# algbio/founderblockgraphs

Measured on AMD Instinct MI355X. Metric: MSA columns segmented/sec, higher is better.
Workload: dtype u32

## Files before the change

### founderblockgraphs_amd/csrc/ctx.hip

```cpp
#include "fbg_internal.h"
#include <chrono>
#include <stdarg.h>
#include <stdio.h>
#include <ctype.h>
#include <string.h>
#include <algorithm>
#include <atomic>
#include <thread>
#include <vector>

static std::string g_global_err;

int fbg_fail(fbg_ctx *ctx, int code, const char *fmt, ...)
{
    char buf[1024];
    va_list ap;
    va_start(ap, fmt);
    vsnprintf(buf, sizeof(buf), fmt, ap);
    va_end(ap);
    if (ctx) ctx->err = buf; else g_global_err = buf;
    return code;
}

int fbg_reserve(fbg_ctx *ctx, DevBuf &b, size_t bytes)
{
    if (bytes == 0) bytes = 256;
    if (b.cap >= bytes) return FBG_OK;
    const auto t_begin = std::chrono::steady_clock::now();
    if (b.p) {
        FBG_HIP_TRY(ctx, hipStreamSynchronize(ctx->stream));
        FBG_HIP_TRY(ctx, hipFree(b.p));
        ctx->held_bytes -= b.cap;
        b.p = nullptr; b.cap = 0;
    }
    size_t want = (bytes + 255) & ~(size_t)255;
    hipError_t e = hipMalloc(&b.p, want);
    if (e != hipSuccess) {
        b.p = nullptr;
        return fbg_fail(ctx, FBG_ERR_OOM, "hipMalloc(%zu bytes) failed: %s (context already holds %llu bytes)",
                        want, hipGetErrorString(e), (unsigned long long)ctx->held_bytes);
    }
    b.cap = want;
    ctx->held_bytes += want;
    ctx->alloc_calls++;
    ctx->alloc_us += (uint64_t)std::chrono::duration_cast<std::chrono::microseconds>(std::chrono::steady_clock::now() - t_begin).count();
    if (ctx->opt.poison) FBG_HIP_TRY(ctx, hipMemsetAsync(b.p, (int)(ctx->opt.poison & 255), want, ctx->stream));
    return FBG_OK;
}

void fbg_release(fbg_ctx *ctx, DevBuf &b)
{
    if (b.p) {
        (void)hipFree(b.p);
        ctx->held_bytes -= b.cap;
        b.p = nullptr; b.cap = 0;
    }
}

#define FBG_STAGE_SLOT (8u << 20)
#define FBG_STAGE_SLOTS 16
#define FBG_STAGE_MIN (32u << 20)

static bool host_pointer_is_pinned(const void *p)
{
    hipPointerAttribute_t at;
    const hipError_t e = hipPointerGetAttributes(&at, p);
    if (e != hipSuccess) { (void)hipGetLastError(); return false; }
    return at.type == hipMemoryTypeHost;
}

static int stager_ready(fbg_ctx *ctx)
{
    Stager &s = ctx->stager;
    if (s.base) return FBG_OK;
    FBG_HIP_TRY(ctx, hipHostMalloc(&s.base, (size_t)FBG_STAGE_SLOT * FBG_STAGE_SLOTS, hipHostMallocDefault));
    s.slot_bytes = FBG_STAGE_SLOT; s.nslots = FBG_STAGE_SLOTS;
    s.ev = new hipEvent_t[s.nslots];
    for (int i = 0; i < s.nslots; i++) FBG_HIP_TRY(ctx, hipEventCreateWithFlags(&s.ev[i], hipEventDisableTiming));
    FBG_HIP_TRY(ctx, hipStreamCreateWithFlags(&s.stream, hipStreamNonBlocking));
    return FBG_OK;
}

static int staged_copy(fbg_ctx *ctx, void *dst, const void *src, size_t bytes, bool to_device)
{
    FBG_HIP_TRY(ctx, hipSetDevice(ctx->device));
    FBG_HIP_TRY(ctx, hipStreamSynchronize(ctx->stream));
    const void *host = to_device ? src : dst;
    if (bytes < FBG_STAGE_MIN || host_pointer_is_pinned(host)) {
        FBG_HIP_TRY(ctx, hipMemcpyAsync(dst, src, bytes, to_device ? hipMemcpyHostToDevice : hipMemcpyDeviceToHost, ctx->stream));
        FBG_HIP_TRY(ctx, hipStreamSynchronize(ctx->stream));
        return FBG_OK;
    }
    FBG_TRY(stager_ready(ctx));
    Stager &s = ctx->stager;
    const size_t nchunks = (bytes + s.slot_bytes - 1) / s.slot_bytes;
    unsigned hw = std::thread::hardware_concurrency();
    int T = (int)std::min<size_t>(std::min<unsigned>(std::max(2u, hw / 2), 8u), nchunks);
    if (T > s.nslots / 2) T = s.nslots / 2;
    std::atomic<int> failed{0};
    auto worker = [&](int t) {
        if (hipSetDevice(ctx->device) != hipSuccess) { failed = 1; return; }
        const int slots[2] = {t, t + T};
        uint8_t *pins[2] = {static_cast<uint8_t *>(s.base) + (size_t)slots[0] * s.slot_bytes,
                            static_cast<uint8_t *>(s.base) + (size_t)slots[1] * s.slot_bytes};
        if (to_device) {
            size_t k = 0;
            for (size_t c = (size_t)t; c < nchunks && !failed; c += (size_t)T, k++) {
                const int w = (int)(k & 1);
                const size_t off = c * s.slot_bytes, len = std::min(s.slot_bytes, bytes - off);
                if (k >= 2 && hipEventSynchronize(s.ev[slots[w]]) != hipSuccess) { failed = 1; return; }
                memcpy(pins[w], static_cast<const uint8_t *>(src) + off, len);
                if (hipMemcpyAsync(static_cast<uint8_t *>(dst) + off, pins[w], len, hipMemcpyHostToDevice, s.stream) != hipSuccess ||
                    hipEventRecord(s.ev[slots[w]], s.stream) != hipSuccess) { failed = 1; return; }
            }
        } else {
            auto issue = [&](size_t c, int w) {
                const size_t off = c * s.slot_bytes, len = std::min(s.slot_bytes, bytes - off);
                return hipMemcpyAsync(pins[w], static_cast<const uint8_t *>(src) + off, len, hipMemcpyDeviceToHost, s.stream) == hipSuccess &&
                       hipEventRecord(s.ev[slots[w]], s.stream) == hipSuccess;
            };
            if ((size_t)t < nchunks && !issue((size_t)t, 0)) { failed = 1; return; }
            size_t k = 0;
            for (size_t c = (size_t)t; c < nchunks && !failed; c += (size_t)T, k++) {
                const int w = (int)(k & 1);
                if (c + (size_t)T < nchunks && !issue(c + (size_t)T, w ^ 1)) { failed = 1; return; }
                if (hipEventSynchronize(s.ev[slots[w]]) != hipSuccess) { failed = 1; return; }
                const size_t off = c * s.slot_bytes, len = std::min(s.slot_bytes, bytes - off);
                memcpy(static_cast<uint8_t *>(dst) + off, pins[w], len);
            }
        }
    };
    std::vector<std::thread> th;
    for (int t = 1; t < T; t++) th.emplace_back(worker, t);
    worker(0);
    for (auto &t : th) t.join();
    FBG_HIP_TRY(ctx, hipStreamSynchronize(s.stream));
    if (failed) return fbg_fail(ctx, FBG_ERR_HIP, "staged %s copy of %zu bytes failed: %s", to_device ? "host-to-device" : "device-to-host",
                                bytes, hipGetErrorString(hipGetLastError()));
    return FBG_OK;
}

int fbg_upload(fbg_ctx *ctx, void *d_dst, const void *h_src, size_t bytes) { return staged_copy(ctx, d_dst, h_src, bytes, true); }
int fbg_download(fbg_ctx *ctx, void *h_dst, const void *d_src, size_t bytes) { return staged_copy(ctx, h_dst, d_src, bytes, false); }

int fbg_stage_begin(fbg_ctx *ctx, int stage)
{
    StageTimer &t = ctx->timers[stage];
    if (!t.start) {
        FBG_HIP_TRY(ctx, hipEventCreate(&t.start));
        FBG_HIP_TRY(ctx, hipEventCreate(&t.stop));
    }
    t.recorded = false;
    FBG_HIP_TRY(ctx, hipEventRecord(t.start, ctx->stream));
    return FBG_OK;
}

int fbg_stage_end(fbg_ctx *ctx, int stage, int launches)
{
    StageTimer &t = ctx->timers[stage];
    FBG_HIP_TRY(ctx, hipEventRecord(t.stop, ctx->stream));
    t.recorded = true;
    t.launches = launches;
    return FBG_OK;
}

struct OptKey { const char *name; int64_t FbgOptions::*field; };
static const OptKey g_opt_keys[] = {
    {"no_ranked", &FbgOptions::no_ranked}, {"no_packed", &FbgOptions::no_packed}, {"force_wide", &FbgOptions::force_wide},
    {"full_keys", &FbgOptions::full_keys}, {"no_msd_sort", &FbgOptions::no_msd_sort}, {"msd_min", &FbgOptions::msd_min},
    {"bp_min", &FbgOptions::bp_min}, {"record_scatter", &FbgOptions::record_scatter}, {"lcp_text", &FbgOptions::lcp_text},
    {"no_aux_stream", &FbgOptions::no_aux_stream}, {"rank_no_threshold", &FbgOptions::rank_no_threshold},
    {"dp_literal", &FbgOptions::dp_literal}, {"dp_wave", &FbgOptions::dp_wave}, {"dp_safe_window", &FbgOptions::dp_safe_window},
    {"dp_tile", &FbgOptions::dp_tile}, {"pure_scan", &FbgOptions::pure_scan}, {"gapped_rank", &FbgOptions::gapped_rank}, {"part_tricks_off", &FbgOptions::part_tricks_off}, {"msd_sample_bins", &FbgOptions::msd_sample_bins}, {"msd_min_force", &FbgOptions::msd_min_force}, {"msd_probe", &FbgOptions::msd_probe}, {"msd_xcd", &FbgOptions::msd_xcd}, {"rank_no_lean", &FbgOptions::rank_no_lean}, {"no_stream_upload", &FbgOptions::no_stream_upload},
    {"span_scan", &FbgOptions::span_scan}, {"span_key_flags", &FbgOptions::span_key_flags}, {"span_slow_split", &FbgOptions::span_slow_split}, {"poison", &FbgOptions::poison}, {"dpw_matrix", &FbgOptions::dpw_matrix}, {"dp_chain1", &FbgOptions::dp_chain1},
};

static void options_from_env(FbgOptions &o)
{
    auto env = [](const std::string &name) -> const char * { return getenv(name.c_str()); };
    const char *dbg = env("FBG_DEBUG_ENV");
    if (!dbg || strcmp(dbg, "1") != 0) return;
    for (const OptKey &k : g_opt_keys) {
        std::string name = "FBG_";
        for (const char *c = k.name; *c; c++) name += (char)toupper((unsigned char)*c);
        if (const char *v = env(name)) o.*(k.field) = *v ? strtoll(v, nullptr, 10) : 1;
    }
}

extern "C" {

int fbg_set_option(fbg_ctx *ctx, const char *key, int64_t value)
{
    if (!ctx || !key) return FBG_ERR_INVALID;
    for (const OptKey &k : g_opt_keys)
        if (strcmp(k.name, key) == 0) { ctx->opt.*(k.field) = value; return FBG_OK; }
    return fbg_fail(ctx, FBG_ERR_INVALID, "fbg_set_option: unknown key '%s'", key);
}

int fbg_get_option(const fbg_ctx *ctx, const char *key, int64_t *value)
{
    if (!ctx || !key || !value) return FBG_ERR_INVALID;
    for (const OptKey &k : g_opt_keys)
        if (strcmp(k.name, key) == 0) { *value = ctx->opt.*(k.field); return FBG_OK; }
    if (strcmp(key, "grs_threshold") == 0) { *value = ctx->grs_t; return FBG_OK; }
    if (strcmp(key, "grs_redone") == 0) { *value = (int64_t)ctx->grs_redone; return FBG_OK; }
    if (strcmp(key, "dp_kind") == 0) { *value = ctx->dp_kind; return FBG_OK; }
    if (strcmp(key, "msd_decline") == 0) { *value = ctx->msd_decline; return FBG_OK; }
    if (strcmp(key, "pass1_ahead") == 0) { *value = ctx->pass1_ahead; return FBG_OK; }
    if (strcmp(key, "alloc_calls") == 0) { *value = (int64_t)ctx->alloc_calls; return FBG_OK; }
    if (strcmp(key, "alloc_us") == 0) { *value = (int64_t)ctx->alloc_us; return FBG_OK; }
    if (strcmp(key, "span_decline") == 0) { *value = ctx->sp_decline; return FBG_OK; }
    if (strcmp(key, "span_key_flags_used") == 0) { *value = (ctx->index_valid && ctx->granked && ctx->spanned && ctx->sp_key_flags_sorted) ? 1 : 0; return FBG_OK; }
    if (strcmp(key, "span_scan_used") == 0) { *value = (ctx->index_valid && ctx->granked && ctx->spanned) ? 1 : 0; return FBG_OK; }
    if (strcmp(key, "span_scan_work") == 0) { *value = (int64_t)ctx->sp_work; return FBG_OK; }
    if (strcmp(key, "span_groups") == 0) { *value = (int64_t)ctx->sp_G; return FBG_OK; }
    if (strcmp(key, "span_odd_groups") == 0) { *value = (int64_t)ctx->sp_n_odd[0] + ctx->sp_n_odd[1] + ctx->sp_n_odd[2] + ctx->sp_n_odd[3]; return FBG_OK; }
    if (strcmp(key, "span_irregular") == 0) { *value = (int64_t)ctx->sp_n_irr; return FBG_OK; }
    if (strcmp(key, "span_chain") == 0) { *value = (int64_t)ctx->sp_chain_n; return FBG_OK; }
    if (strcmp(key, "span_slow_groups") == 0) { *value = (int64_t)ctx->sp_slow_n; return FBG_OK; }
    if (strncmp(key, "span_dbg", 8) == 0 && key[8] >= '0' && key[8] <= '7' && !key[9]) {
        unsigned long long v = 0;
        if (hipStreamSynchronize(ctx->stream) != hipSuccess || ctx->scalars.cap < 256 * 8 ||
            hipMemcpy(&v, (const unsigned long long *)ctx->scalars.p + 208 + 24 + (key[8] - '0'), 8, hipMemcpyDeviceToHost) != hipSuccess) return FBG_ERR_HIP;
        *value = (int64_t)v;
        return FBG_OK;
    }
    if (strcmp(key, "index_kind") == 0) {
        *value = !ctx->index_valid ? -1 : ctx->part_active ? 3 : ctx->granked ? 2 : ctx->ranked ? 1 : 0;
        return FBG_OK;
    }
    return FBG_ERR_INVALID;
}

void *fbg_host_alloc(uint64_t bytes)
{
    void *p = nullptr;
    if (hipHostMalloc(&p, bytes ? bytes : 1, hipHostMallocDefault) != hipSuccess) { (void)hipGetLastError(); return nullptr; }
    return p;
}
void fbg_host_free(void *p) { if (p) (void)hipHostFree(p); }

int fbg_ctx_create(int device, fbg_ctx **out)
{
    if (!out) return FBG_ERR_INVALID;
    *out = nullptr;
    int count = 0;
    hipError_t e = hipGetDeviceCount(&count);
    if (e != hipSuccess || count <= 0)
        return fbg_fail(nullptr, FBG_ERR_NO_DEVICE,
                        "no HIP device visible (%s); libfbg_hip has no CPU fallback",
                        e != hipSuccess ? hipGetErrorString(e) : "device count 0");
    if (device < 0 || device >= count)
        return fbg_fail(nullptr, FBG_ERR_INVALID, "device %d out of range (0..%d)", device, count - 1);
    e = hipSetDevice(device);
    if (e != hipSuccess) return fbg_fail(nullptr, FBG_ERR_HIP, "hipSetDevice: %s", hipGetErrorString(e));
    fbg_ctx *ctx = new fbg_ctx();
    ctx->device = device;
    options_from_env(ctx->opt);
    e = hipStreamCreateWithFlags(&ctx->stream, hipStreamNonBlocking);
    if (e != hipSuccess) {
        delete ctx;
        return fbg_fail(nullptr, FBG_ERR_HIP, "hipStreamCreate: %s", hipGetErrorString(e));
    }
    ctx->own_stream = true;
    *out = ctx;
    return FBG_OK;
}

void fbg_ctx_destroy(fbg_ctx *ctx)
{
    if (!ctx) return;
    (void)hipSetDevice(ctx->device);
    (void)hipStreamSynchronize(ctx->stream);
    DevBuf *bufs[] = {&ctx->msa_own, &ctx->text, &ctx->pos, &ctx->tot, &ctx->segtab, &ctx->exc_scratch, &ctx->prow, &ctx->igrow, &ctx->rec,
                      &ctx->xlist, &ctx->gmax, &ctx->excol, &ctx->xslot, &ctx->xbits, &ctx->exc, &ctx->colT, &ctx->keysA, &ctx->keysB, &ctx->valsA, &ctx->valsB, &ctx->grp, &ctx->flags,
                      &ctx->list, &ctx->tie_list, &ctx->big_groups, &ctx->kargs, &ctx->msd_w, &ctx->msd_v, &ctx->tmp, &ctx->small, &ctx->scalars, &ctx->dp_a, &ctx->dp_b, &ctx->dp_c,
                      &ctx->dp_d, &ctx->dp_e, &ctx->dp_f, &ctx->dp_g, &ctx->dp_h, &ctx->io_a, &ctx->io_b,
                      &ctx->io_c, &ctx->io_d, &ctx->bt_up, &ctx->bt_dep, &ctx->ps_a, &ctx->ps_b, &ctx->ps_c, &ctx->ps_d,
                      &ctx->ps_e, &ctx->ps_f, &ctx->ps_g, &ctx->ps_h, &ctx->gwin, &ctx->gbits, &ctx->gwin_rows,
                      &ctx->sp_cells, &ctx->sp_flagT, &ctx->sp_cwin, &ctx->sp_tiles, &ctx->sp_gstart, &ctx->sp_gcol, &ctx->sp_gflags, &ctx->sp_rstart, &ctx->sp_rid,
                      &ctx->sp_gplo, &ctx->sp_gphi, &ctx->sp_gval, &ctx->sp_odd, &ctx->sp_irr, &ctx->sp_chain, &ctx->sp_slow, &ctx->sp_mins};
    for (DevBuf *b : bufs) fbg_release(ctx, *b);
    if (ctx->up_stream) {
        (void)hipStreamSynchronize(ctx->up_stream);
        for (auto &e : ctx->up_ev) if (e) (void)hipEventDestroy(e);
        (void)hipStreamDestroy(ctx->up_stream);
    }
    for (auto &t : ctx->timers) {
        if (t.start) (void)hipEventDestroy(t.start);
        if (t.stop) (void)hipEventDestroy(t.stop);
    }
    if (ctx->stager.base) {
        for (int i = 0; i < ctx->stager.nslots; i++) (void)hipEventDestroy(ctx->stager.ev[i]);
        delete[] ctx->stager.ev;
        (void)hipStreamDestroy(ctx->stager.stream);
        (void)hipHostFree(ctx->stager.base);
    }
    if (ctx->aux_fork) (void)hipEventDestroy(ctx->aux_fork);
    if (ctx->aux_join) (void)hipEventDestroy(ctx->aux_join);
    if (ctx->aux) (void)hipStreamDestroy(ctx->aux);
    if (ctx->own_stream) (void)hipStreamDestroy(ctx->stream);
    delete ctx;
}

const char *fbg_last_error(const fbg_ctx *ctx) { return ctx ? ctx->err.c_str() : g_global_err.c_str(); }

int fbg_set_stream(fbg_ctx *ctx, void *hip_stream)
{
    if (!ctx) return FBG_ERR_INVALID;
    FBG_HIP_TRY(ctx, hipStreamSynchronize(ctx->stream));
    if (ctx->own_stream) { (void)hipStreamDestroy(ctx->stream); ctx->own_stream = false; }
    if (hip_stream) {
        ctx->stream = (hipStream_t)hip_stream;
    } else {
        FBG_HIP_TRY(ctx, hipStreamCreateWithFlags(&ctx->stream, hipStreamNonBlocking));
        ctx->own_stream = true;
    }
    return FBG_OK;
}

int fbg_stage_ms(fbg_ctx *ctx, int stage, float *ms, int *launches)
{
    if (!ctx || stage < 0 || stage >= FBG_STAGE_COUNT) return FBG_ERR_INVALID;
    StageTimer &t = ctx->timers[stage];
    if (ms) *ms = 0.f;
    if (launches) *launches = 0;
    if (!t.recorded) return FBG_OK;
    FBG_HIP_TRY(ctx, hipEventSynchronize(t.stop));
    float v = 0.f;
    FBG_HIP_TRY(ctx, hipEventElapsedTime(&v, t.start, t.stop));
    if (ms) *ms = v;
    if (launches) *launches = t.launches;
    return FBG_OK;
}

uint64_t fbg_device_bytes(const fbg_ctx *ctx) { return ctx ? ctx->held_bytes : 0; }

int fbg_release_scratch(fbg_ctx *ctx)
{
    if (!ctx) return FBG_ERR_INVALID;
    FBG_HIP_TRY(ctx, hipSetDevice(ctx->device));
    FBG_HIP_TRY(ctx, hipStreamSynchronize(ctx->stream));
    const bool sorted_in_A = (ctx->ranked || ctx->granked) && ctx->rk_keys == ctx->keysA.as<uint64_t>();
    DevBuf *bufs[] = {sorted_in_A ? &ctx->keysB : &ctx->keysA, &ctx->valsA, &ctx->grp, &ctx->flags, &ctx->list, &ctx->tie_list, &ctx->msd_w, &ctx->msd_v,
                      &ctx->tmp, &ctx->dp_a, &ctx->dp_b, &ctx->dp_c, &ctx->dp_d, &ctx->dp_e, &ctx->dp_f,
                      &ctx->dp_g, &ctx->dp_h, &ctx->ps_a, &ctx->ps_b, &ctx->ps_c, &ctx->ps_d, &ctx->ps_e, &ctx->ps_f,
                      &ctx->ps_g, &ctx->ps_h, &ctx->sp_cells, &ctx->sp_flagT, &ctx->sp_tiles};
    for (DevBuf *b : bufs) fbg_release(ctx, *b);
    return FBG_OK;
}

int fbg_sync(fbg_ctx *ctx)
{
    if (!ctx) return FBG_ERR_INVALID;
    FBG_HIP_TRY(ctx, hipStreamSynchronize(ctx->stream));
    return FBG_OK;
}

static int check_dims(fbg_ctx *ctx, uint64_t m, uint64_t n)
{
    if (!ctx) return FBG_ERR_INVALID;
    if (m == 0 || n == 0) return fbg_fail(ctx, FBG_ERR_INVALID, "empty MSA (m=%llu, n=%llu)",
                                          (unsigned long long)m, (unsigned long long)n);
    if (n >= (1ull << 31) || m * (n + 1) + 1 >= (1ull << 40))
        return fbg_fail(ctx, FBG_ERR_TOO_LARGE, "MSA of %llu x %llu cells is beyond this engine (n < 2^31, text < 2^40)",
                        (unsigned long long)m, (unsigned long long)n);
    return FBG_OK;
}

int fbg_msa_set_device(fbg_ctx *ctx, const uint8_t *d_msa, uint64_t m, uint64_t n)
{
    FBG_TRY(check_dims(ctx, m, n));
    if (!d_msa) return fbg_fail(ctx, FBG_ERR_INVALID, "null MSA pointer");
    ctx->d_msa = d_msa; ctx->m = m; ctx->n = n; ctx->index_valid = false;
    return FBG_OK;
}

int fbg_msa_load_host(fbg_ctx *ctx, const uint8_t *msa, uint64_t m, uint64_t n)
{
    FBG_TRY(check_dims(ctx, m, n));
    if (!msa) return fbg_fail(ctx, FBG_ERR_INVALID, "null MSA pointer");
    FBG_HIP_TRY(ctx, hipSetDevice(ctx->device));
    FBG_TRY(fbg_reserve(ctx, ctx->msa_own, m * n));
    FBG_TRY(fbg_upload(ctx, ctx->msa_own.p, msa, m * n));
    ctx->d_msa = ctx->msa_own.as<uint8_t>(); ctx->m = m; ctx->n = n; ctx->index_valid = false;
    return FBG_OK;
}

int fbg_index_build(fbg_ctx *ctx, int reversed, const uint8_t *ignore_chars, uint64_t ignore_len)
{
    if (!ctx) return FBG_ERR_INVALID;
    if (!ctx->d_msa) return fbg_fail(ctx, FBG_ERR_INVALID, "fbg_index_build: no MSA set");
    FBG_HIP_TRY(ctx, hipSetDevice(ctx->device));
    for (int st : {FBG_STAGE_SORT_PASS1, FBG_STAGE_SORT_PASS2, FBG_STAGE_SORT_PASS3, FBG_STAGE_RANK_KERNEL}) {
        ctx->timers[st].recorded = false;
        ctx->timers[st].launches = 0;
    }
    ctx->index_valid = false;
    ctx->granked = false;
    ctx->spanned = false;
    ctx->gpart = false;
    ctx->reversed = reversed ? 1 : 0;
    FBG_TRY(fbg_build_text(ctx, reversed ? nullptr : ignore_chars, reversed ? 0 : ignore_len));
    FBG_TRY(fbg_suffix_sort(ctx));
    FBG_TRY(fbg_neighbour_lcp(ctx));
    if (ctx->N > 1500000000ull) {
        size_t free_b = 0, total_b = 0;
        FBG_HIP_TRY(ctx, hipMemGetInfo(&free_b, &total_b));
        if (free_b < total_b / 2) FBG_TRY(fbg_release_scratch(ctx));
    }
    ctx->index_valid = true;
    return FBG_OK;
}

int fbg_part_index_build(fbg_ctx *ctx, int reversed, int part, int nparts, void *d_blob, int *ok)
{
    return fbg_part_index_build_ignore(ctx, reversed, part, nparts, nullptr, 0, d_blob, ok);
}

int fbg_part_index_build_ignore(fbg_ctx *ctx, int reversed, int part, int nparts, const uint8_t *ignore_chars, uint64_t ignore_len, void *d_blob, int *ok)
{
    if (!ctx) return FBG_ERR_INVALID;
    if (!ctx->d_msa) return fbg_fail(ctx, FBG_ERR_INVALID, "fbg_part_index_build: no MSA set");
    if (!d_blob || !ok || nparts < 1 || part < 0 || part >= nparts || (ignore_len && !ignore_chars))
        return fbg_fail(ctx, FBG_ERR_INVALID, "fbg_part_index_build: bad arguments");
    FBG_HIP_TRY(ctx, hipSetDevice(ctx->device));
    ctx->index_valid = false;
    ctx->ranked = false;
    ctx->granked = false;
    ctx->spanned = false;
    ctx->reversed = reversed ? 1 : 0;
    ctx->gpart = false;
    ctx->allow_wide = true;
    const int rc = fbg_build_text(ctx, reversed ? nullptr : ignore_chars, reversed ? 0 : ignore_len);
    ctx->allow_wide = false;
    FBG_TRY(rc);
    return fbg_part_sort(ctx, part, nparts, static_cast<uint8_t *>(d_blob), ok);
}

int fbg_part_scan(fbg_ctx *ctx, const void *d_blobs, uint32_t *d_gmax, int *ok)
{
    if (!ctx) return FBG_ERR_INVALID;
    if (!ctx->part_active || ctx->index_valid)
        return fbg_fail(ctx, FBG_ERR_INVALID, "fbg_part_scan needs fbg_part_index_build first");
    if (!d_blobs || !d_gmax || !ok) return fbg_fail(ctx, FBG_ERR_INVALID, "fbg_part_scan: bad arguments");
    FBG_HIP_TRY(ctx, hipSetDevice(ctx->device));
    if (ctx->gpart) return fbg_grs_part_scan(ctx, static_cast<const uint8_t *>(d_blobs), d_gmax, ok);
    return fbg_rank_part_runs(ctx, static_cast<const uint8_t *>(d_blobs), d_gmax, ok);
}

int fbg_part_finish(fbg_ctx *ctx, const uint32_t *d_gmax, int *ok)
{
    if (!ctx) return FBG_ERR_INVALID;
    if (!ctx->part_active || ctx->index_valid)
        return fbg_fail(ctx, FBG_ERR_INVALID, "fbg_part_finish needs fbg_part_scan first");
    if (!d_gmax || !ok) return fbg_fail(ctx, FBG_ERR_INVALID, "fbg_part_finish: bad arguments");
    FBG_HIP_TRY(ctx, hipSetDevice(ctx->device));
    uint32_t verdict = 1;
    FBG_HIP_TRY(ctx, hipMemcpyAsync(ctx->gmax.p, d_gmax, (ctx->n + 1) * 4, hipMemcpyDeviceToDevice, ctx->stream));
    FBG_HIP_TRY(ctx, hipMemcpyAsync(&verdict, d_gmax + ctx->n, 4, hipMemcpyDeviceToHost, ctx->stream));
    FBG_HIP_TRY(ctx, hipStreamSynchronize(ctx->stream));
    *ok = verdict == 0;
    if (*ok) {
        uint64_t unfilled = 0;
        if (ctx->gpart) FBG_TRY(fbg_grs_part_unfilled(ctx, &unfilled));
        else FBG_TRY(fbg_rank_part_unfilled(ctx, &unfilled));
        if (unfilled) { *ok = 2; return FBG_OK; }
        ctx->n_exc = 0; ctx->index_valid = true;
        if (ctx->gpart) ctx->granked = true; else ctx->ranked = true;
    }
    return FBG_OK;
}

int fbg_part_rescan(fbg_ctx *ctx, uint32_t *d_gmax)
{
    if (!ctx) return FBG_ERR_INVALID;
    if (!ctx->part_active || ctx->index_valid)
        return fbg_fail(ctx, FBG_ERR_INVALID, "fbg_part_rescan follows a fbg_part_finish that returned *ok = 2");
    if (!d_gmax) return fbg_fail(ctx, FBG_ERR_INVALID, "fbg_part_rescan: bad arguments");
    FBG_HIP_TRY(ctx, hipSetDevice(ctx->device));
    uint32_t verdict = 0;
    if (ctx->gpart) { FBG_TRY(fbg_grs_part_rescan(ctx)); verdict = ctx->grs_part_failed ? 1u : 0u; }
    else FBG_TRY(fbg_rank_part_rescan(ctx));
    FBG_HIP_TRY(ctx, hipMemcpyAsync(d_gmax, ctx->gmax.p, (ctx->n + 1) * 4, hipMemcpyDeviceToDevice, ctx->stream));
    FBG_HIP_TRY(ctx, hipMemcpyAsync(d_gmax + ctx->n, &verdict, 4, hipMemcpyHostToDevice, ctx->stream));
    FBG_HIP_TRY(ctx, hipStreamSynchronize(ctx->stream));
    return FBG_OK;
}

int fbg_scan_f(fbg_ctx *ctx, uint64_t x0, uint64_t x1, int disable_tricks, uint64_t *d_f)
{
    if (!ctx) return FBG_ERR_INVALID;
    if (!ctx->index_valid || ctx->reversed)
        return fbg_fail(ctx, FBG_ERR_INVALID, "fbg_scan_f needs fbg_index_build(reversed=0) first");
    if (x0 > x1 || x1 > ctx->n || !d_f) return fbg_fail(ctx, FBG_ERR_INVALID, "fbg_scan_f: bad column range");
    FBG_HIP_TRY(ctx, hipSetDevice(ctx->device));
    return fbg_scan_columns(ctx, x0, x1, FBG_SCAN_F, disable_tricks, d_f);
// ... 238 lines not shown
```

### founderblockgraphs_amd/csrc/fbg_internal.h

```cpp
#pragma once
#include <cstring>
#include <cstdlib>
#include <hip/hip_runtime.h>
#include <stdint.h>
#include <string>
#include "../../include/fbg_hip.h"

#define FBG_WAVE 64

struct DevBuf {
    void *p = nullptr;
    size_t cap = 0;
    template <class T> T *as() const { return reinterpret_cast<T *>(p); }
};

struct Stager {
    void *base = nullptr;
    size_t slot_bytes = 0;
    int nslots = 0;
    hipEvent_t *ev = nullptr;
    hipStream_t stream = nullptr;
};

struct StageTimer {
    hipEvent_t start = nullptr, stop = nullptr;
    bool recorded = false;
    int launches = 0;
};

struct FbgOptions {
    int64_t no_ranked = 0, no_packed = 0, force_wide = 0, full_keys = 0, no_msd_sort = 0, msd_min = -1, bp_min = -1,
            record_scatter = 0, lcp_text = 0, no_aux_stream = 0, rank_no_threshold = 0, dp_literal = 0, dp_wave = 0,
            dp_safe_window = 0, dp_tile = 0, pure_scan = 0, gapped_rank = 0, part_tricks_off = 0, msd_sample_bins = 0, msd_min_force = 0, msd_probe = 0, msd_xcd = -1, rank_no_lean = 0, no_stream_upload = 0,
            span_scan = 0, span_key_flags = 0, span_slow_split = 0, poison = 0, dpw_matrix = 0, dp_chain1 = 0;
};

struct fbg_ctx {
    int device = 0;
    FbgOptions opt;
    hipStream_t stream = nullptr;
    bool own_stream = false;
    hipStream_t aux = nullptr;
    hipEvent_t aux_fork = nullptr, aux_join = nullptr;
    bool aux_pending = false;
    std::string err;
    uint64_t held_bytes = 0;
    Stager stager;

    const uint8_t *d_msa = nullptr;
    DevBuf msa_own;
    uint64_t m = 0, n = 0;

    const uint8_t *up_host = nullptr;
    hipStream_t up_stream = nullptr;
    hipEvent_t up_ev[9] = {};
    bool pre_pass1 = false;
    uint64_t pre_symbols[4] = {0, 0, 0, 0};
    alignas(16) unsigned char pre_state[768];
    uint64_t pre_tiles = 0;
    int pass1_ahead = 0;

    bool index_valid = false;
    int reversed = 0;
    bool gapfree = true;
    bool have_ignore = false;
    uint64_t N = 0;
    uint64_t byte_hist[256] = {0};
    bool allow_wide = false;
    uint32_t mp = 0;
    DevBuf text;
    DevBuf pos, tot;
    DevBuf segtab;
    DevBuf prow;
    DevBuf igrow;
    DevBuf rec;
    uint32_t *sa_ptr = nullptr;
    bool lcp_from_keys = false;
    DevBuf colT;
    DevBuf xlist;
    bool ranked = false;
    DevBuf gmax, excol, xslot;
    DevBuf xbits;
    DevBuf exc_scratch;
    DevBuf exc;
    uint32_t n_exc = 0;
    bool granked = false;
    int grs_tricks_off = 0;
    bool grs_skip = false;
    uint32_t grs_ign_lo = 0, grs_ign_hi = 0;
    DevBuf gwin;
    DevBuf gbits;
    DevBuf gwin_rows;
    const uint64_t *grs_ebits = nullptr;
    bool grs_flagged = false;
    bool pairs_similar = false;
    bool grs_ties_done = false;
    bool gpart = false;
    bool grs_part_failed = false;
    uint32_t grs_t = 1;
    uint64_t grs_redone = 0;
    bool spanned = false;
    DevBuf sp_cells;
    DevBuf sp_flagT;
    bool sp_key_flags = false;
    uint64_t alloc_calls = 0, alloc_us = 0;
    int sp_decline = 0;
    bool sp_key_flags_sorted = false;
    DevBuf sp_cwin;
    DevBuf sp_tiles, sp_gstart, sp_gcol, sp_gflags, sp_rstart, sp_rid, sp_gplo, sp_gphi, sp_gval, sp_odd, sp_irr, sp_chain, sp_slow, sp_mins;
    uint32_t sp_chain_n = 0, sp_slow_n = 0;
    uint64_t sp_G = 0, sp_R = 0, sp_n_irr = 0, sp_work = 0;
    uint32_t sp_n_odd[4] = {0, 0, 0, 0}, sp_odd_cap = 0;
    const uint32_t *sort_payload = nullptr;
    int64_t msd_decline = -1;
    int dp_kind = -1;
    bool cells_built = false;
    uint8_t ignore_tab[256] = {0};
    uint64_t *rk_keys = nullptr;
    int rk_b = 0, rk_key_bits = 0, rk_K = 0;
    int rk_layout = 0, rk_pb = 0;
    bool part_active = false;
    int part = 0, nparts = 1;
    uint64_t part_count = 0;
    uint64_t part_T = 0;
    uint32_t part_gmin = 0;

    DevBuf keysA, keysB, valsA, valsB, grp, flags, list, tie_list, big_groups, tmp, small, scalars;
    DevBuf kargs;
    alignas(16) unsigned char kargs_host[512];
    DevBuf msd_w, msd_v;
    DevBuf dp_a, dp_b, dp_c, dp_d, dp_e, dp_f, dp_g, dp_h, io_a, io_b, io_c, io_d;
    DevBuf bt_up, bt_dep;
    DevBuf ps_a, ps_b, ps_c, ps_d, ps_e, ps_f, ps_g, ps_h;

    StageTimer timers[FBG_STAGE_COUNT];
};

int fbg_fail(fbg_ctx *ctx, int code, const char *fmt, ...);
#define FBG_HIP_TRY(ctx, expr)                                                              \
    do {                                                                                    \
        hipError_t e_ = (expr);                                                             \
        if (e_ != hipSuccess)                                                               \
            return fbg_fail((ctx), e_ == hipErrorOutOfMemory ? FBG_ERR_OOM : FBG_ERR_HIP,   \
                            "%s failed: %s (%s:%d)", #expr, hipGetErrorString(e_), __FILE__, \
                            __LINE__);                                                      \
    } while (0)
#define FBG_TRY(expr)                \
    do {                             \
        int rc_ = (expr);            \
        if (rc_ != FBG_OK) return rc_; \
    } while (0)

int fbg_reserve(fbg_ctx *ctx, DevBuf &b, size_t bytes);
int fbg_upload(fbg_ctx *ctx, void *d_dst, const void *h_src, size_t bytes);
int fbg_download(fbg_ctx *ctx, void *h_dst, const void *d_src, size_t bytes);
void fbg_release(fbg_ctx *ctx, DevBuf &b);
int fbg_stage_begin(fbg_ctx *ctx, int stage);
int fbg_stage_end(fbg_ctx *ctx, int stage, int launches);

#define FBG_SLOTS_PAIRS 0
#define FBG_SLOTS_PACKED 1
#define FBG_SLOTS_WIDE 2
struct KeyGeom {
    int b = 0, K = 0, key_bits = 0;
    bool compact = false, packed = false;
    bool wide = false;
    int pb = 0;
    const uint8_t *d_code = nullptr;
};

int fbg_build_text(fbg_ctx *ctx, const uint8_t *ignore, uint64_t ignore_len);
int fbg_suffix_sort(fbg_ctx *ctx);
int fbg_neighbour_lcp(fbg_ctx *ctx);
int fbg_rank_scan_try(fbg_ctx *ctx, uint64_t *keys, uint32_t *vals, const KeyGeom &g, int *done);
int fbg_pure_scan_try(fbg_ctx *ctx, uint64_t *keys, uint32_t *vals, const KeyGeom &g, int *done);
int fbg_rank_finish(fbg_ctx *ctx, uint64_t x0, uint64_t x1, int mode, int disable_tricks, uint64_t *d_out);
int fbg_rank_materialize(fbg_ctx *ctx, uint32_t *d_sa, uint32_t *d_isa, uint32_t *d_pl, uint32_t *d_pr);
#define FBG_STAGE_RANKSCAN FBG_STAGE_TILE
int fbg_grs_prepare(fbg_ctx *ctx, int *launches);
int fbg_grs_part_classify(fbg_ctx *ctx, uint64_t *keys, uint32_t *vals, uint64_t count, const KeyGeom &g, int eligible, uint8_t *d_blob, int *ok);
int fbg_grs_part_scan(fbg_ctx *ctx, const uint8_t *d_blobs, uint32_t *d_gmax, int *ok);
int fbg_grs_part_unfilled(fbg_ctx *ctx, uint64_t *unfilled);
int fbg_grs_part_rescan(fbg_ctx *ctx);
int fbg_grs_strip(fbg_ctx *ctx, uint32_t *vals);
int fbg_grs_try(fbg_ctx *ctx, uint64_t *keys, uint32_t *vals, const KeyGeom &g, int *done);
int fbg_grs_finish(fbg_ctx *ctx, uint64_t x0, uint64_t x1, int disable_tricks, uint64_t *d_out, int *ok);
int fbg_grs_materialize(fbg_ctx *ctx, uint32_t *d_sa, uint32_t *d_isa, uint32_t *d_pl, uint32_t *d_pr);
bool fbg_span_eligible(fbg_ctx *ctx, const KeyGeom &g);
bool fbg_span_key_flags(fbg_ctx *ctx, KeyGeom &g);
int fbg_span_prepare(fbg_ctx *ctx, const KeyGeom &g, int *launches);
int fbg_span_try(fbg_ctx *ctx, uint64_t *keys, uint32_t *vals, const KeyGeom &g, int *done);
int fbg_span_rescan(fbg_ctx *ctx, int disable_tricks, int *ok);
int fbg_build_cell_tables(fbg_ctx *ctx);
int fbg_key_setup(fbg_ctx *ctx, bool compact, KeyGeom *g, int *launches);
int fbg_rank_part_classify(fbg_ctx *ctx, uint64_t *keys, uint32_t *vals, uint64_t count, const KeyGeom &g, int pre_ok,
                           uint8_t *d_blob, int *ok);
int fbg_rank_part_runs(fbg_ctx *ctx, const uint8_t *d_blobs, uint32_t *d_gmax, int *ok);
int fbg_rank_part_unfilled(fbg_ctx *ctx, uint64_t *unfilled);
int fbg_rank_part_rescan(fbg_ctx *ctx);
int fbg_part_sort(fbg_ctx *ctx, int part, int nparts, uint8_t *d_blob, int *ok);
int fbg_msd_sort(fbg_ctx *ctx, const KeyGeom &g, uint64_t **sorted, int *ok, int *launches);
int fbg_msd_pre_begin(fbg_ctx *ctx, int *ok);
int fbg_msd_pre_pass1(fbg_ctx *ctx, uint64_t avail);
bool fbg_msd_pre_geom(fbg_ctx *ctx, KeyGeom *g);
int fbg_msd_sort_part(fbg_ctx *ctx, const KeyGeom &g, uint64_t lo, uint64_t hi, int nohi, int nparts, uint64_t out_offset,
                      uint64_t *count, int *ok, int *launches);
int fbg_sample_sort_pairs(fbg_ctx *ctx, const KeyGeom &g, int *ok, int *launches);
int fbg_scan_columns(fbg_ctx *ctx, uint64_t x0, uint64_t x1, int mode, int disable_tricks,
                     uint64_t *d_out);
int fbg_dp_minmax(fbg_ctx *ctx, const uint64_t *d_f, uint64_t n, uint64_t *d_boundaries,
                  uint64_t *count_out, uint64_t *d_mml, uint64_t *d_bt);
int fbg_dp_repeatfree(fbg_ctx *ctx, const uint64_t *d_v, uint64_t n, uint64_t *d_s,
                      uint64_t *d_prev, uint64_t *d_boundaries, uint64_t *count_out);
int fbg_gapped_v_from_f(fbg_ctx *ctx, const uint64_t *d_f, uint64_t n, uint64_t *d_v);
int fbg_dp_gapped(fbg_ctx *ctx, const uint64_t *d_v, uint64_t n, uint64_t *d_s, uint64_t *d_prev,
                  uint64_t *d_boundaries, uint64_t *count_out);

#define FBG_SCAN_F 0
#define FBG_SCAN_V 1

static inline unsigned fbg_blocks(uint64_t work, unsigned per_block, unsigned cap = 0x7fffffffu)
{
    uint64_t b = (work + per_block - 1) / per_block;
    if (b < 1) b = 1;
    if (b > cap) b = cap;
    return (unsigned)b;
}
```

### founderblockgraphs_amd/csrc/msd_sort.hip

```cpp
#include "fbg_internal.h"
#include "msd_keys.h"
#include <rocprim/rocprim.hpp>
#include <algorithm>
#include <cmath>

#define MSD_DIG 9
#define MSD_NB (1 << MSD_DIG)
#define MSD_THREADS 1024
#define MSD_TILE (MSD_THREADS * MSD_ITEMS)
#define MSD_FN_THREADS 512
#define MSD_FN_CAP 4096
#define MSD_FN_ITEMS (MSD_FN_CAP / MSD_FN_THREADS)
#define MSD_FN_BITS 11
#define MSD_FN_BINS (1 << MSD_FN_BITS)
#define MSD_BIG_THREADS 1024
#define MSD_BIG_CAP 16384
#define MSD_ARENA (1u << 20)

struct MsdArgs {
    const uint8_t *T;
    uint64_t N;
    const uint8_t *code;
    int b, K, pb, kb;
    uint64_t *buf1;
    uint64_t cap1;
    int xs;
    uint64_t segcap;
    unsigned long long *count1;
    const uint32_t *tile_start;
    uint64_t tile0;
    uint32_t tiles2, tiles2_x;
    uint64_t *buf2;
    uint32_t *count2;
    const unsigned long long *off;
    uint64_t *out;
    uint32_t *arena_sb;
    uint64_t *arena_w;
    unsigned long long *arena_count;
    uint32_t arena_cap;
    unsigned long long *flag;
};

__device__ __forceinline__ void msd_scan_and_reserve(uint32_t *cnt, uint32_t *loff, uint32_t *gdelta, uint32_t *wsum,
                                                     unsigned long long *cursor_d, bool wide_cursor, uint32_t *cursor32_d)
{
    const uint32_t lane = threadIdx.x & 63, wv = threadIdx.x >> 6;
    const uint32_t c = threadIdx.x < MSD_NB ? cnt[threadIdx.x] : 0u;
    uint32_t inc = c;
#pragma unroll
    for (int d = 1; d < 64; d <<= 1) { const uint32_t o = __shfl_up(inc, d, 64); if ((int)lane >= d) inc += o; }
    if (lane == 63) wsum[wv] = inc;
    __syncthreads();
    uint32_t pre = 0;
    for (uint32_t q = 0; q < wv; q++) pre += wsum[q];
    if (threadIdx.x < MSD_NB) {
        loff[threadIdx.x] = pre + inc - c;
        unsigned long long g = 0;
        if (c) g = wide_cursor ? atomicAdd(cursor_d, (unsigned long long)c) : (unsigned long long)atomicAdd(cursor32_d, c);
        gdelta[threadIdx.x] = (uint32_t)g - (pre + inc - c);
    }
    __syncthreads();
}

template <bool FULL>
__device__ __forceinline__ void msd_pack_split_body(const MsdArgs &a, uint64_t *buf, const uint8_t *cd, uint32_t *cnt, uint32_t *loff, uint32_t *gdelta,
                                                    uint32_t *wsum)
{
    uint8_t *tile = reinterpret_cast<uint8_t *>(buf);
    const int b = a.b, K = a.K;
    const uint64_t base = ((uint64_t)blockIdx.x + a.tile0) * MSD_TILE;
    msd_load_tile<MSD_TILE, FULL>(tile, cd, a.T, a.N, base);
    __syncthreads();
    const int t0 = threadIdx.x * MSD_ITEMS;
    uint64_t w[MSD_ITEMS];
    msd_build_keys(tile, t0, b, K, w);
    __syncthreads();
    uint32_t rk[MSD_ITEMS];
    const int dshift = a.kb - MSD_DIG;
#pragma unroll
    for (int i = 0; i < MSD_ITEMS; i++) {
        const uint64_t p = base + t0 + i;
        const bool ok = FULL || p < a.N;
        rk[i] = ok ? atomicAdd(&cnt[(uint32_t)(w[i] >> dshift)], 1u) : 0xffffffffu;
        w[i] = (w[i] << a.pb) | p;
    }
    __syncthreads();
    const uint32_t xq = a.xs > 1 ? (blockIdx.x & (uint32_t)(a.xs - 1)) : 0u;
    msd_scan_and_reserve(cnt, loff, gdelta, wsum, a.count1 + (threadIdx.x < MSD_NB ? threadIdx.x * a.xs + xq : 0), true, nullptr);
    const int wshift = a.pb + dshift;
    uint64_t *const obase = a.buf1 + xq * a.segcap;
#pragma unroll
    for (int i = 0; i < MSD_ITEMS; i++)
        if (FULL || rk[i] != 0xffffffffu) buf[loff[(uint32_t)(w[i] >> wshift)] + rk[i]] = w[i];
    __syncthreads();
    const uint32_t have = FULL ? (uint32_t)MSD_TILE : (uint32_t)min((uint64_t)MSD_TILE, a.N - base);
    bool over = false;
#pragma unroll
    for (int r = 0; r < MSD_ITEMS; r++) {
        const uint32_t j = threadIdx.x + r * MSD_THREADS;
        if (FULL || j < have) {
            const uint64_t x = buf[j];
            const uint32_t d = (uint32_t)(x >> wshift);
            const uint32_t at = j + gdelta[d];
            if (at < a.segcap) obase[(uint64_t)d * a.cap1 + at] = x;
            else over = true;
        }
    }
    if (over) atomicOr(a.flag, 2ull);
}

__global__ __launch_bounds__(MSD_THREADS) void k_msd_pack_split(MsdArgs a)
{
    __shared__ uint64_t buf[MSD_TILE];
    __shared__ uint8_t cd[256];
    __shared__ uint32_t cnt[MSD_NB], loff[MSD_NB];
    __shared__ uint32_t gdelta[MSD_NB];
    __shared__ uint32_t wsum[MSD_THREADS / 64];
    if (threadIdx.x < 256) cd[threadIdx.x] = a.code[threadIdx.x];
    if (threadIdx.x < MSD_NB) cnt[threadIdx.x] = 0;
    __syncthreads();
    msd_pack_split_body<false>(a, buf, cd, cnt, loff, gdelta, wsum);
}

__global__ __launch_bounds__(1024) void k_msd_tiles(const unsigned long long *__restrict__ count1, uint64_t segcap, uint32_t nseg,
                                                    uint32_t *__restrict__ tile_start, unsigned long long *__restrict__ flag)
{
    __shared__ uint32_t wsum[16];
    const uint32_t lane = threadIdx.x & 63, wv = threadIdx.x >> 6;
    uint32_t t[4], tot = 0;
#pragma unroll
    for (int q = 0; q < 4; q++) {
        const uint32_t s = threadIdx.x * 4 + q;
        t[q] = 0;
        if (s < nseg) {
            const unsigned long long c = count1[s] < segcap ? count1[s] : segcap;
            if (count1[s] > segcap) atomicOr(flag, 4ull);
            t[q] = (uint32_t)((c + MSD_TILE - 1) / MSD_TILE);
        }
        tot += t[q];
    }
    uint32_t inc = tot;
#pragma unroll
    for (int d = 1; d < 64; d <<= 1) { const uint32_t o = __shfl_up(inc, d, 64); if ((int)lane >= d) inc += o; }
    if (lane == 63) wsum[wv] = inc;
    __syncthreads();
    uint32_t pre = inc - tot;
    for (uint32_t q = 0; q < wv; q++) pre += wsum[q];
#pragma unroll
    for (int q = 0; q < 4; q++) {
        const uint32_t s = threadIdx.x * 4 + q;
        if (s < nseg) tile_start[s] = pre;
        pre += t[q];
        if (s + 1 == nseg) tile_start[nseg] = pre;
    }
}

template <bool FULL>
__device__ __forceinline__ void msd_split_body(const MsdArgs &a, uint64_t *buf, uint32_t *cnt, uint32_t *loff, uint32_t *gdelta, uint32_t *wsum,
                                               const uint64_t *__restrict__ in, uint32_t have, uint32_t seg)
{
    const int wshift = a.pb + a.kb - 2 * MSD_DIG;
    uint64_t w[MSD_ITEMS];
    uint32_t rk[MSD_ITEMS];
#pragma unroll
    for (int r = 0; r < MSD_ITEMS; r++) {
        const uint32_t j = threadIdx.x + r * MSD_THREADS;
        w[r] = (FULL || j < have) ? in[j] : 0ull;
    }
#pragma unroll
    for (int r = 0; r < MSD_ITEMS; r++) {
        const uint32_t j = threadIdx.x + r * MSD_THREADS;
        rk[r] = (FULL || j < have) ? atomicAdd(&cnt[(uint32_t)(w[r] >> wshift) & (MSD_NB - 1)], 1u) : 0u;
    }
    __syncthreads();
    msd_scan_and_reserve(cnt, loff, gdelta, wsum, nullptr, false,
                         a.count2 + (size_t)seg * MSD_NB + (threadIdx.x < MSD_NB ? threadIdx.x : 0));
#pragma unroll
    for (int r = 0; r < MSD_ITEMS; r++) {
        const uint32_t j = threadIdx.x + r * MSD_THREADS;
        if (FULL || j < have) buf[loff[(uint32_t)(w[r] >> wshift) & (MSD_NB - 1)] + rk[r]] = w[r];
    }
    __syncthreads();
    uint64_t *const obase = a.buf2 + (uint64_t)seg * MSD_NB * MSD_FN_CAP;
#pragma unroll
    for (int r = 0; r < MSD_ITEMS; r++) {
        const uint32_t j = threadIdx.x + r * MSD_THREADS;
        if (FULL || j < have) {
            const uint64_t x = buf[j];
            const uint32_t d = (uint32_t)(x >> wshift) & (MSD_NB - 1);
            const uint32_t at = j + gdelta[d];
            if (at < MSD_FN_CAP) obase[d * MSD_FN_CAP + at] = x;
            else {
                const unsigned long long e = atomicAdd(a.arena_count, 1ull);
                if (e < a.arena_cap) { a.arena_sb[e] = seg * MSD_NB + d; a.arena_w[e] = x; }
                else atomicOr(a.flag, 8ull);
            }
        }
    }
}

__global__ __launch_bounds__(MSD_THREADS) void k_msd_split(MsdArgs a)
{
    __shared__ uint64_t buf[MSD_TILE];
    __shared__ uint32_t cnt[MSD_NB], loff[MSD_NB];
    __shared__ uint32_t gdelta[MSD_NB];
    __shared__ uint32_t wsum[MSD_THREADS / 64];
    const uint32_t tile = a.tiles2_x ? (blockIdx.x & 7u) * a.tiles2_x + (blockIdx.x >> 3) : blockIdx.x;
    if (tile >= a.tiles2) return;
    uint32_t lo = 0, hi = MSD_NB * (uint32_t)a.xs;
    while (hi - lo > 1) { const uint32_t mid = (lo + hi) / 2; if (a.tile_start[mid] <= tile) lo = mid; else hi = mid; }
    const uint32_t seg = lo / (uint32_t)a.xs;
    const uint64_t segn = min((uint64_t)a.count1[lo], a.segcap);
    const uint64_t first = (uint64_t)(tile - a.tile_start[lo]) * MSD_TILE;
    const uint32_t have = (uint32_t)min((uint64_t)MSD_TILE, segn - first);
    const uint64_t *in = a.buf1 + (uint64_t)seg * a.cap1 + (uint64_t)(lo % (uint32_t)a.xs) * a.segcap + first;
    if (threadIdx.x < MSD_NB) cnt[threadIdx.x] = 0;
    __syncthreads();
    if (__builtin_amdgcn_readfirstlane((int)have) == MSD_TILE) msd_split_body<true>(a, buf, cnt, loff, gdelta, wsum, in, have, seg);
    else msd_split_body<false>(a, buf, cnt, loff, gdelta, wsum, in, have, seg);
}

__global__ void k_msd_widen(const uint32_t *__restrict__ count2, unsigned long long *__restrict__ wide, uint64_t cnt)
{
    const uint64_t i = (uint64_t)blockIdx.x * blockDim.x + threadIdx.x;
    if (i < cnt) wide[i] = count2[i];
}

#define MSD_BIG_BIN 192
#define MSD_LOW_BITS 10
template <int CAP, int THREADS>
__device__ __forceinline__ void msd_finish_sort(uint64_t *buf, uint32_t *cnt, uint32_t *loff, uint32_t *wsum, uint64_t (&w)[CAP / THREADS],
                                                uint32_t have, int fshift, uint32_t fmask, int lowbits, uint32_t *sub, uint16_t *biglist,
                                                uint32_t *nbig_lds)
{
    constexpr int ITEMS = CAP / THREADS;
    for (int i = threadIdx.x; i < MSD_FN_BINS; i += THREADS) cnt[i] = 0;
    __syncthreads();
    uint32_t rk[ITEMS];
#pragma unroll
    for (int r = 0; r < ITEMS; r++) {
        const uint32_t j = threadIdx.x + r * THREADS;
        rk[r] = j < have ? atomicAdd(&cnt[(uint32_t)(w[r] >> fshift) & fmask], 1u) : 0u;
    }
    __syncthreads();
    {
        constexpr int PER = MSD_FN_BINS / THREADS > 0 ? MSD_FN_BINS / THREADS : 1;
        const uint32_t lane = threadIdx.x & 63, wv = threadIdx.x >> 6;
        const bool mine = threadIdx.x * PER < MSD_FN_BINS;
        uint32_t c[PER], tot = 0;
#pragma unroll
        for (int q = 0; q < PER; q++) { c[q] = mine ? cnt[threadIdx.x * PER + q] : 0u; tot += c[q]; }
        uint32_t inc = tot;
#pragma unroll
        for (int d = 1; d < 64; d <<= 1) { const uint32_t o = __shfl_up(inc, d, 64); if ((int)lane >= d) inc += o; }
        if (lane == 63) wsum[wv] = inc;
        __syncthreads();
        uint32_t pre = inc - tot;
        for (uint32_t q = 0; q < wv; q++) pre += wsum[q];
        if (mine) {
#pragma unroll
            for (int q = 0; q < PER; q++) { loff[threadIdx.x * PER + q] = pre; pre += c[q]; }
        }
    }
    __syncthreads();
#pragma unroll
    for (int r = 0; r < ITEMS; r++) {
        const uint32_t j = threadIdx.x + r * THREADS;
        if (j < have) buf[loff[(uint32_t)(w[r] >> fshift) & fmask] + rk[r]] = w[r];
    }
    __syncthreads();
    uint32_t nbig = 0;
    if (lowbits >= 1 && lowbits <= MSD_LOW_BITS) {
        if (threadIdx.x == 0) *nbig_lds = 0;
        __syncthreads();
        for (int i = threadIdx.x; i < MSD_FN_BINS; i += THREADS)
            if (cnt[i] > MSD_BIG_BIN) { const uint32_t e = atomicAdd(nbig_lds, 1u); biglist[e] = (uint16_t)i; }
        __syncthreads();
        nbig = *nbig_lds;
    }
    const uint32_t lowmask = (1u << (lowbits > 0 ? lowbits : 1)) - 1;
    for (uint32_t e = 0; e < nbig; e++) {
        const uint32_t bbin = biglist[e], b0 = loff[bbin];
        for (uint32_t i = threadIdx.x; i <= lowmask; i += THREADS) sub[i] = 0;
        __syncthreads();
        uint32_t idx[ITEMS];
#pragma unroll
        for (int r = 0; r < ITEMS; r++) {
            const uint32_t j = threadIdx.x + r * THREADS;
            idx[r] = 0;
            if (j < have && ((uint32_t)(w[r] >> fshift) & fmask) == bbin) idx[r] = atomicAdd(&sub[(uint32_t)(w[r] >> (fshift - lowbits)) & lowmask], 1u);
        }
        __syncthreads();
        {
            constexpr int PER = (1 << MSD_LOW_BITS) / THREADS > 0 ? (1 << MSD_LOW_BITS) / THREADS : 1;
            const uint32_t lane = threadIdx.x & 63, wv = threadIdx.x >> 6;
            uint32_t c[PER], tot = 0;
#pragma unroll
            for (int q = 0; q < PER; q++) { const uint32_t i = threadIdx.x * PER + q; c[q] = i <= lowmask ? sub[i] : 0u; tot += c[q]; }
            uint32_t inc = tot;
#pragma unroll
            for (int d = 1; d < 64; d <<= 1) { const uint32_t o = __shfl_up(inc, d, 64); if ((int)lane >= d) inc += o; }
            if (lane == 63) wsum[wv] = inc;
            __syncthreads();
            uint32_t pre = inc - tot;
            for (uint32_t q = 0; q < wv; q++) pre += wsum[q];
#pragma unroll
            for (int q = 0; q < PER; q++) { const uint32_t i = threadIdx.x * PER + q; if (i <= lowmask) sub[i] = pre; pre += c[q]; }
        }
        __syncthreads();
#pragma unroll
        for (int r = 0; r < ITEMS; r++) {
            const uint32_t j = threadIdx.x + r * THREADS;
            if (j < have && ((uint32_t)(w[r] >> fshift) & fmask) == bbin)
                rk[r] = b0 + sub[(uint32_t)(w[r] >> (fshift - lowbits)) & lowmask] + idx[r];
        }
        __syncthreads();
    }
    if (nbig) {
#pragma unroll
        for (int r = 0; r < ITEMS; r++) {
            const uint32_t j = threadIdx.x + r * THREADS;
            if (j < have && cnt[(uint32_t)(w[r] >> fshift) & fmask] > MSD_BIG_BIN) buf[rk[r]] = w[r];
        }
        __syncthreads();
    }
#pragma unroll
    for (int r = 0; r < ITEMS; r++) {
        const uint32_t j = threadIdx.x + r * THREADS;
        if (j < have) {
            const uint64_t y = buf[j];
            const uint32_t bin = (uint32_t)(y >> fshift) & fmask;
            const uint32_t b0 = loff[bin], c = cnt[bin];
            uint32_t at = j;
            if (!(c > MSD_BIG_BIN && (nbig || lowbits == 0))) {
                uint32_t smaller = 0;
                for (uint32_t q = 0; q < c; q++) smaller += buf[b0 + q] < y ? 1u : 0u;
                at = b0 + smaller;
            }
            w[r] = y;
            rk[r] = at;
        }
    }
    __syncthreads();
#pragma unroll
    for (int r = 0; r < ITEMS; r++) {
        const uint32_t j = threadIdx.x + r * THREADS;
        if (j < have) buf[rk[r]] = w[r];
    }
    __syncthreads();
}

template <int CAP, int THREADS>
__device__ __forceinline__ void msd_finish_body(uint64_t *buf, uint32_t *cnt, uint32_t *loff, uint32_t *wsum, const uint64_t *in_a,
                                                uint32_t n_a, const uint64_t *in_b, uint32_t have, uint64_t *out, int fshift,
                                                uint32_t fmask, int lowbits, uint32_t *sub, uint16_t *biglist, uint32_t *nbig_lds)
{
    constexpr int ITEMS = CAP / THREADS;
    uint64_t w[ITEMS];
#pragma unroll
    for (int r = 0; r < ITEMS; r++) {
        const uint32_t j = threadIdx.x + r * THREADS;
        w[r] = j < have ? (j < n_a ? in_a[j] : in_b[j - n_a]) : ~0ull;
    }
    msd_finish_sort<CAP, THREADS>(buf, cnt, loff, wsum, w, have, fshift, fmask, lowbits, sub, biglist, nbig_lds);
#pragma unroll
    for (int r = 0; r < ITEMS; r++) {
        const uint32_t j = threadIdx.x + r * THREADS;
        if (j < have) out[j] = buf[j];
    }
}

__global__ __launch_bounds__(MSD_FN_THREADS) void k_msd_finish(MsdArgs a, int fshift, uint32_t fmask)
{
    __shared__ uint64_t buf[MSD_FN_CAP];
    __shared__ uint32_t cnt[MSD_FN_BINS], loff[MSD_FN_BINS];
    __shared__ uint32_t wsum[MSD_FN_THREADS / 64];
    __shared__ uint32_t sub[1 << MSD_LOW_BITS];
    __shared__ uint16_t biglist[MSD_FN_CAP / MSD_BIG_BIN + 1];
    __shared__ uint32_t nbig_lds;
    const uint32_t have = a.count2[blockIdx.x];
    if (have == 0 || have > MSD_FN_CAP) return;
    const uint64_t *in = a.buf2 + (uint64_t)blockIdx.x * MSD_FN_CAP;
    msd_finish_body<MSD_FN_CAP, MSD_FN_THREADS>(buf, cnt, loff, wsum, in, have, in, have, a.out + a.off[blockIdx.x], fshift, fmask,
                                                fshift - a.pb, sub, biglist, &nbig_lds);
}

__global__ __launch_bounds__(MSD_BIG_THREADS) void k_msd_finish_big(MsdArgs a, const uint32_t *__restrict__ sb_sorted,
                                                                    const uint64_t *__restrict__ w_sorted, uint32_t entries,
                                                                    int fshift, uint32_t fmask)
{
    __shared__ uint64_t buf[MSD_BIG_CAP];
    __shared__ uint32_t cnt[MSD_FN_BINS], loff[MSD_FN_BINS];
    __shared__ uint32_t wsum[MSD_BIG_THREADS / 64];
    __shared__ uint32_t sub[1 << MSD_LOW_BITS];
    __shared__ uint16_t biglist[MSD_BIG_CAP / MSD_BIG_BIN + 1];
    __shared__ uint32_t nbig_lds;
    const uint32_t e = blockIdx.x;
    if (e >= entries) return;
    const uint32_t sb = sb_sorted[e];
    if (e > 0 && sb_sorted[e - 1] == sb) return;
    const uint32_t have = a.count2[sb];
    if (have > MSD_BIG_CAP || have <= MSD_FN_CAP) { if (threadIdx.x == 0) atomicOr(a.flag, 16ull); return; }
    msd_finish_body<MSD_BIG_CAP, MSD_BIG_THREADS>(buf, cnt, loff, wsum, a.buf2 + (uint64_t)sb * MSD_FN_CAP, MSD_FN_CAP, w_sorted + e, have,
                                                  a.out + a.off[sb], fshift, fmask, fshift - a.pb, sub, biglist, &nbig_lds);
}

struct MsdPlan {
    KeyGeom g;
    MsdArgs a;
    uint64_t nsub;
    uint32_t nseg;
    int rest, fbits, xcd;
    uint32_t *tile_start;
    unsigned long long *off, *flag;
};
static_assert(sizeof(MsdPlan) <= sizeof(((fbg_ctx *)nullptr)->pre_state), "room for the plan of a sort begun ahead");

static int msd_plan(fbg_ctx *ctx, const KeyGeom &g, MsdPlan *p, int *ok)
{
    *ok = 0;
    const uint64_t N = ctx->N;
    const int rest = g.key_bits - 2 * MSD_DIG;
    const uint64_t min_n = ctx->opt.msd_min >= 0 ? (uint64_t)ctx->opt.msd_min : (1ull << 24);
    if (!g.packed || !g.compact || N < min_n || rest < 1 || ctx->opt.no_msd_sort) return FBG_OK;
    if (N >= (1ull << 31)) return FBG_OK;
    const int fbits = rest < MSD_FN_BITS ? rest : MSD_FN_BITS;
    if (fbits < 6) return FBG_OK;
    hipStream_t st = ctx->stream;
    const int xcd = ctx->opt.msd_xcd < 0 ? 3 : (int)ctx->opt.msd_xcd;
    const int xs = (xcd & 2) ? 8 : 1;
    const uint64_t cap1 = (N / MSD_NB + N / (4 * MSD_NB) + 65536) & ~127ull;
    const uint64_t nsub = (uint64_t)MSD_NB * MSD_NB;
    if (N / nsub + N / (32 * nsub) + 64 > MSD_FN_CAP) return FBG_OK;
    FBG_TRY(fbg_reserve(ctx, ctx->keysA, (size_t)MSD_NB * cap1 * 8));
    FBG_TRY(fbg_reserve(ctx, ctx->keysB, (size_t)nsub * MSD_FN_CAP * 8));
    const uint32_t nseg = MSD_NB * (uint32_t)xs;
    FBG_TRY(fbg_reserve(ctx, ctx->dp_a, (size_t)nseg * 8 + ((size_t)nseg + 1) * 4 + 64));
    FBG_TRY(fbg_reserve(ctx, ctx->dp_b, nsub * 4));
    FBG_TRY(fbg_reserve(ctx, ctx->dp_c, (nsub + 1) * 8));
    FBG_TRY(fbg_reserve(ctx, ctx->dp_d, (size_t)MSD_ARENA * 4 * 2));
    FBG_TRY(fbg_reserve(ctx, ctx->dp_e, (size_t)MSD_ARENA * 8 * 2));
    unsigned long long *flag = ctx->scalars.as<unsigned long long>() + 100;
    MsdArgs &a = p->a;
    a.T = ctx->text.as<uint8_t>(); a.N = N; a.code = g.d_code; a.b = g.b; a.K = g.K; a.pb = g.pb; a.kb = g.key_bits;
    a.buf1 = ctx->keysA.as<uint64_t>(); a.cap1 = cap1; a.xs = xs; a.segcap = cap1 / xs;
    a.tile0 = 0; a.tiles2 = 0; a.tiles2_x = 0;
    a.count1 = ctx->dp_a.as<unsigned long long>();
    p->tile_start = reinterpret_cast<uint32_t *>(ctx->dp_a.as<uint8_t>() + (size_t)nseg * 8);
    a.tile_start = p->tile_start;
    a.buf2 = ctx->keysB.as<uint64_t>();
    a.count2 = ctx->dp_b.as<uint32_t>();
    p->off = ctx->dp_c.as<unsigned long long>();
    a.off = p->off;
    a.out = ctx->keysA.as<uint64_t>();
    a.flag = flag;
    a.arena_sb = ctx->dp_d.as<uint32_t>(); a.arena_w = ctx->dp_e.as<uint64_t>(); a.arena_count = flag + 1; a.arena_cap = MSD_ARENA;
    p->g = g; p->nsub = nsub; p->nseg = nseg; p->rest = rest; p->fbits = fbits; p->xcd = xcd; p->flag = flag;
    FBG_HIP_TRY(ctx, hipMemsetAsync(flag, 0, 16, st));
    FBG_HIP_TRY(ctx, hipMemsetAsync(a.count1, 0, (size_t)nseg * 8, st));
    FBG_HIP_TRY(ctx, hipMemsetAsync(a.count2, 0, nsub * 4, st));
    *ok = 1;
    return FBG_OK;
}

int fbg_msd_pre_begin(fbg_ctx *ctx, int *ok)
{
    *ok = 0;
    if (ctx->have_ignore || ctx->reversed || ctx->opt.no_ranked) return FBG_OK;
    int launches = 0;
    KeyGeom g;
    FBG_TRY(fbg_key_setup(ctx, true, &g, &launches));
    MsdPlan plan;
    int good = 0;
    FBG_TRY(msd_plan(ctx, g, &plan, &good));
    if (!good) return FBG_OK;
    for (int w = 0; w < 4; w++) ctx->pre_symbols[w] = 0;
    for (int b = 0; b < 256; b++) if (ctx->byte_hist[b]) ctx->pre_symbols[b >> 6] |= 1ull << (b & 63);
    memcpy(ctx->pre_state, &plan, sizeof(plan));
    ctx->pre_tiles = 0;
    *ok = 1;
    return FBG_OK;
}

int fbg_msd_pre_pass1(fbg_ctx *ctx, uint64_t avail)
{
    MsdPlan plan;
    memcpy(&plan, ctx->pre_state, sizeof(plan));
    const uint64_t N = plan.a.N;
    const uint64_t upto = avail >= N ? (N + MSD_TILE - 1) / MSD_TILE : (avail >= 64 ? (avail - 64) / MSD_TILE : 0);
    if (upto <= ctx->pre_tiles) return FBG_OK;
    plan.a.tile0 = ctx->pre_tiles;
    hipLaunchKernelGGL(k_msd_pack_split, dim3((unsigned)(upto - ctx->pre_tiles)), dim3(MSD_THREADS), 0, ctx->stream, plan.a);
    ctx->pre_tiles = upto;
    return FBG_OK;
}

bool fbg_msd_pre_geom(fbg_ctx *ctx, KeyGeom *g)
{
    if (!ctx->pre_pass1) return false;
    MsdPlan plan;
    memcpy(&plan, ctx->pre_state, sizeof(plan));
    *g = plan.g;
    return true;
}

int fbg_msd_sort(fbg_ctx *ctx, const KeyGeom &g, uint64_t **sorted, int *ok, int *launches)
{
    *ok = 0;
    ctx->msd_decline = 1;
    const uint64_t N = ctx->N;
    hipStream_t st = ctx->stream;
    MsdPlan plan;
    const bool ahead = ctx->pre_pass1;
    ctx->pre_pass1 = false;
    ctx->pass1_ahead = ahead ? 1 : 0;
    if (ahead) memcpy(&plan, ctx->pre_state, sizeof(plan));
    else {
        int good = 0;
        FBG_TRY(msd_plan(ctx, g, &plan, &good));
        if (!good) return FBG_OK;
    }
    MsdArgs &a = plan.a;
    const uint64_t nsub = plan.nsub;
    const uint32_t nseg = plan.nseg;
    const int rest = plan.rest, fbits = plan.fbits, xcd = plan.xcd;
    uint32_t *tile_start = plan.tile_start;
    unsigned long long *off = plan.off, *flag = plan.flag;
    if (!ahead) {
        FBG_TRY(fbg_stage_begin(ctx, FBG_STAGE_SORT_PASS1));
        hipLaunchKernelGGL(k_msd_pack_split, dim3(fbg_blocks(N, MSD_TILE)), dim3(MSD_THREADS), 0, st, a);
        FBG_TRY(fbg_stage_end(ctx, FBG_STAGE_SORT_PASS1, 1));
    }
    hipLaunchKernelGGL(k_msd_tiles, dim3(1), dim3(1024), 0, st, a.count1, a.segcap, nseg, tile_start, flag);
    uint32_t tiles2 = 0;
    unsigned long long h_flag = 0;
    FBG_HIP_TRY(ctx, hipMemcpyAsync(&tiles2, tile_start + nseg, 4, hipMemcpyDeviceToHost, st));
    FBG_HIP_TRY(ctx, hipMemcpyAsync(&h_flag, flag, 8, hipMemcpyDeviceToHost, st));
    FBG_HIP_TRY(ctx, hipStreamSynchronize(st));
    *launches += 2;
    ctx->msd_decline = (int64_t)h_flag;
    if (h_flag != 0 || tiles2 == 0) return FBG_OK;
    a.tiles2 = tiles2;
    a.tiles2_x = (xcd & 1) ? (tiles2 + 7) / 8 : 0;
    const unsigned grid2 = a.tiles2_x ? 8 * a.tiles2_x : tiles2;
    FBG_TRY(fbg_stage_begin(ctx, FBG_STAGE_SORT_PASS2));
    hipLaunchKernelGGL(k_msd_split, dim3(grid2), dim3(MSD_THREADS), 0, st, a);
    FBG_TRY(fbg_stage_end(ctx, FBG_STAGE_SORT_PASS2, 1));
    unsigned long long *wide = reinterpret_cast<unsigned long long *>(ctx->keysA.p);
    hipLaunchKernelGGL(k_msd_widen, dim3(fbg_blocks(nsub, 256)), dim3(256), 0, st, a.count2, wide, nsub);
    {
        size_t bytes = 0;
        hipError_t e = rocprim::exclusive_scan(nullptr, bytes, wide, off, 0ull, (size_t)nsub, rocprim::plus<unsigned long long>(), st);
        if (e != hipSuccess) return fbg_fail(ctx, FBG_ERR_HIP, "rocprim scan size query: %s", hipGetErrorString(e));
        FBG_TRY(fbg_reserve(ctx, ctx->tmp, bytes));
        size_t have = ctx->tmp.cap;
        e = rocprim::exclusive_scan(ctx->tmp.p, have, wide, off, 0ull, (size_t)nsub, rocprim::plus<unsigned long long>(), st);
        if (e != hipSuccess) return fbg_fail(ctx, FBG_ERR_HIP, "rocprim exclusive_scan: %s", hipGetErrorString(e));
    }
    const int fshift = g.pb + rest - fbits;
    const uint32_t fmask = (uint32_t)((1u << fbits) - 1);
    FBG_TRY(fbg_stage_begin(ctx, FBG_STAGE_SORT_PASS3));
    hipLaunchKernelGGL(k_msd_finish, dim3((unsigned)nsub), dim3(MSD_FN_THREADS), 0, st, a, fshift, fmask);
    FBG_TRY(fbg_stage_end(ctx, FBG_STAGE_SORT_PASS3, 1));
    unsigned long long h2[2] = {0, 0};
    FBG_HIP_TRY(ctx, hipMemcpyAsync(h2, flag, 16, hipMemcpyDeviceToHost, st));
    FBG_HIP_TRY(ctx, hipStreamSynchronize(st));
    *launches += 4;
    ctx->msd_decline = (int64_t)h2[0];
    if (h2[0] != 0) return FBG_OK;
    if (h2[1] > 0) {
        const uint32_t entries = (uint32_t)h2[1];
        uint32_t *sb_sorted = a.arena_sb + MSD_ARENA;
        uint64_t *w_sorted = a.arena_w + MSD_ARENA;
        size_t bytes = 0;
        hipError_t e = rocprim::radix_sort_pairs(nullptr, bytes, a.arena_sb, sb_sorted, a.arena_w, w_sorted, (size_t)entries, 0u, 32u, st);
        if (e != hipSuccess) return fbg_fail(ctx, FBG_ERR_HIP, "rocprim sort size query: %s", hipGetErrorString(e));
        FBG_TRY(fbg_reserve(ctx, ctx->tmp, bytes));
        size_t have = ctx->tmp.cap;
        e = rocprim::radix_sort_pairs(ctx->tmp.p, have, a.arena_sb, sb_sorted, a.arena_w, w_sorted, (size_t)entries, 0u, 32u, st);
        if (e != hipSuccess) return fbg_fail(ctx, FBG_ERR_HIP, "rocprim radix_sort_pairs: %s", hipGetErrorString(e));
        hipLaunchKernelGGL(k_msd_finish_big, dim3(entries), dim3(MSD_BIG_THREADS), 0, st, a, sb_sorted, w_sorted, entries, fshift, fmask);
        FBG_HIP_TRY(ctx, hipMemcpyAsync(h2, flag, 16, hipMemcpyDeviceToHost, st));
        FBG_HIP_TRY(ctx, hipStreamSynchronize(st));
        *launches += 2;
        ctx->msd_decline = (int64_t)h2[0];
        if (h2[0] != 0) return FBG_OK;
    }
    FBG_HIP_TRY(ctx, hipGetLastError());
    *sorted = ctx->keysA.as<uint64_t>();
    *ok = 1;
    return FBG_OK;
}
```

### founderblockgraphs_amd/csrc/rank_common.h

```cpp
#pragma once
#include "fbg_internal.h"
#include "text_cmp.h"

#define RS_TG 4

__device__ __forceinline__ uint32_t rs_key_lcp(uint64_t a, uint64_t c, int b, int key_bits)
{
    const uint64_t d = a ^ c;
    const uint32_t bits = (uint32_t)(__clzll((long long)d) - (64 - key_bits));
    const uint32_t inv_b = (65536u + (uint32_t)b - 1) / (uint32_t)b;
    return (bits * inv_b) >> 16;
}

struct RankArgs {
    uint32_t magic32;
    uint64_t magic64;
    uint64_t *keys;
    uint32_t *vals;
    uint64_t pmask;
    int pb;
    const uint8_t *T;
    uint64_t N, n;
    uint64_t Ntext;
    uint64_t own_lo, own_hi;
    int first_part, last_part;
    int part_mode;
    int values_only;
    uint32_t row_len;
    uint32_t g_min;
    int b, key_bits, K, reversed;
    uint32_t *gmax;
    uint32_t *cand;
    uint32_t *blk_count;
    uint32_t region;
    uint32_t *ties;
    uint32_t *tie_count;
    uint32_t tie_region;
    uint2 *pairs;
    uint32_t *pair_count;
    uint32_t *pm;
    uint32_t *big;
    unsigned long long *counters;
};

struct Slot {
    uint64_t key;
    uint64_t pos;
    uint32_t col;
    uint32_t rem;
};

__device__ __forceinline__ uint32_t rs_col_of_rem(const RankArgs &a, uint32_t rem)
{
    return rem == 0 ? (uint32_t)a.n : (a.reversed ? rem - 1 : (uint32_t)a.n - rem);
}
template <int L> struct PosT { typedef uint32_t type; };
template <> struct PosT<FBG_SLOTS_WIDE> { typedef uint64_t type; };
template <int L> __device__ __forceinline__ uint64_t rs_key(const RankArgs &a, uint64_t k) { return a.keys[k] >> a.pb; }
template <int L> __device__ __forceinline__ uint64_t rs_pos_of(const RankArgs &a, uint64_t w, uint32_t v)
{
    if (L == FBG_SLOTS_PACKED) return w & a.pmask;
    if (L == FBG_SLOTS_WIDE) return ((w & a.pmask) << 32) | v;
    return v;
}
template <int L> __device__ __forceinline__ uint64_t rs_pos(const RankArgs &a, uint64_t k)
{
    return rs_pos_of<L>(a, L == FBG_SLOTS_PAIRS ? 0ull : a.keys[k], L == FBG_SLOTS_PACKED ? 0u : a.vals[k]);
}
template <int L> __device__ __forceinline__ void rs_set_pos(const RankArgs &a, uint64_t k, uint64_t p)
{
    if (L == FBG_SLOTS_PACKED) a.keys[k] = (a.keys[k] & ~a.pmask) | p;
    else if (L == FBG_SLOTS_WIDE) { a.keys[k] = (a.keys[k] & ~a.pmask) | (p >> 32); a.vals[k] = (uint32_t)p; }
    else a.vals[k] = (uint32_t)p;
}
template <int L> __device__ __forceinline__ uint32_t rs_rem(const RankArgs &a, uint64_t p)
{
    if (L == FBG_SLOTS_WIDE) {
        uint64_t c = p - __umul64hi(p, a.magic64) * a.row_len;
        if (c >= a.row_len) c -= a.row_len;
        return p == a.Ntext - 1 ? 0u : (uint32_t)(a.n - c);
    }
    const uint32_t p32 = (uint32_t)p;
    uint32_t c = p32 - __umulhi(p32, a.magic32) * a.row_len;
    if (c >= a.row_len) c -= a.row_len;
    return p32 == (uint32_t)(a.Ntext - 1) ? 0u : (uint32_t)a.n - c;
}
template <int L> __device__ __forceinline__ Slot rs_slot(const RankArgs &a, uint64_t k)
{
    Slot s;
    const uint64_t w = a.keys[k];
    s.key = w >> a.pb;
    s.pos = rs_pos_of<L>(a, w, L == FBG_SLOTS_PACKED ? 0u : a.vals[k]);
    s.rem = rs_rem<L>(a, s.pos);
    s.col = rs_col_of_rem(a, s.rem);
    return s;
}
template <int L> __device__ __forceinline__ uint32_t rs_col(const RankArgs &a, uint64_t k)
{
    return rs_col_of_rem(a, rs_rem<L>(a, rs_pos<L>(a, k)));
}

__device__ __forceinline__ void rs_update(const RankArgs &a, uint32_t col, uint32_t g)
{
    if (a.gmax[col] < g) atomicMax(&a.gmax[col], g);
}


__device__ __forceinline__ void rs_append(bool want, uint32_t *counter, uint32_t *list, uint32_t region, uint32_t value)
{
    const unsigned long long mask = __ballot(want);
    if (!mask) return;
    const int lane = threadIdx.x & 63;
    uint32_t base = 0;
    const int leader = __ffsll((long long)mask) - 1;
    if (lane == leader) base = atomicAdd(counter, (uint32_t)__popcll(mask));
    base = __shfl(base, leader, 64);
    if (want) {
        const uint32_t slot = base + (uint32_t)__popcll(mask & ((1ull << lane) - 1));
        if (slot < region) list[(size_t)blockIdx.x * region + slot] = value;
    }
}

#define RS_HALO 8

struct RsLdsView {
    const uint64_t *skey;
    const uint32_t *srem;
    __device__ __forceinline__ uint64_t key(int i) const { return skey[i]; }
    __device__ __forceinline__ uint32_t rem(int i) const { return srem[i]; }
};
struct RsWordView {
    const uint64_t *words;
    const RankArgs *a;
    int lo, hi;
    __device__ __forceinline__ uint64_t word(int i) const { return i >= lo && i < hi ? words[i] : 0ull; }
    __device__ __forceinline__ uint64_t key(int i) const { return word(i) >> a->pb; }
    __device__ __forceinline__ uint32_t rem(int i) const { return rs_rem<FBG_SLOTS_PACKED>(*a, word(i) & a->pmask); }
};

template <class V>
__device__ __forceinline__ void rank_scan_slow(const RankArgs &a, const V &v, const int i,
                                               const int lo_i, const int hi_i, const uint64_t k, bool &want_cand, bool &want_tie)
{
    const uint64_t key = v.key(i);
    const uint32_t rem = v.rem(i);
    const bool has_prev = i > lo_i, has_next = i + 1 < hi_i;
    const uint64_t kp = v.key(i - 1), kn = v.key(i + 1);
    const bool tie = (has_prev && kp == key) || (has_next && kn == key);
    if (tie) {
        int h = i, t = i;
        while (h > lo_i && i - h < RS_TG && v.key(h - 1) == key) h--;
        bool big = h > lo_i && v.key(h - 1) == key;
        while (t + 1 < hi_i && t - i < RS_TG && v.key(t + 1) == key) t++;
        big = big || (t + 1 < hi_i && v.key(t + 1) == key) || t - h + 1 > RS_TG;
        bool simple = !big;
        if (simple && a.part_mode && (k - (uint64_t)(i - h) < a.own_lo + 2 || k + (uint64_t)(t - i) + 2 >= a.own_hi))
            simple = false;
        if (simple) {
            uint32_t cols[RS_TG];
            const int s = t - h + 1;
#pragma unroll
            for (int q = 0; q < RS_TG; q++) {
                cols[q] = 0xffffffffu - (uint32_t)q;
                if (q < s) {
                    cols[q] = v.rem(h + q);
                    if (cols[q] < (uint32_t)a.K) simple = false;
                }
            }
#pragma unroll
            for (int q = 0; q < RS_TG; q++)
#pragma unroll
                for (int r = q + 1; r < RS_TG; r++)
                    if (cols[q] == cols[r]) simple = false;
            if (simple && h > lo_i) {
                if (h - 1 > lo_i && v.key(h - 2) == v.key(h - 1)) simple = false;
                const uint32_t oc = v.rem(h - 1);
#pragma unroll
                for (int q = 0; q < RS_TG; q++)
                    if (cols[q] == oc) simple = false;
            }
            if (simple && t + 1 < hi_i) {
                if (t + 2 < hi_i && v.key(t + 2) == v.key(t + 1)) simple = false;
                const uint32_t oc = v.rem(t + 1);
#pragma unroll
                for (int q = 0; q < RS_TG; q++)
                    if (cols[q] == oc) simple = false;
            }
        }
        if (simple) want_tie = i == h;
        else want_cand = true;
        return;
    }
    if (rem == 0) return;
    const bool edge = a.part_mode && (k < a.own_lo + 2 || k + 2 >= a.own_hi);
    bool run = (has_prev && v.rem(i - 1) == rem) || (has_next && v.rem(i + 1) == rem);
    uint32_t mrp = has_prev ? v.rem(i - 1) : 0u, mrn = has_next ? v.rem(i + 1) : 0u;
    if (has_prev && i - 1 > lo_i && v.key(i - 2) == kp) {
        int j = i - 1, cnt = 0;
        uint32_t mr = 0;
        for (;;) {
            const uint32_t rj = v.rem(j);
            mr = max(mr, rj);
            run = run || rj == rem;
            cnt++;
            if (j == lo_i || v.key(j - 1) != kp) break;
            if (cnt == RS_TG) { run = true; break; }
            j--;
        }
        mrp = mr;
    }
    if (has_next && i + 2 < hi_i && v.key(i + 2) == kn) {
        int j = i + 1, cnt = 0;
        uint32_t mr = 0;
        for (;;) {
            const uint32_t rj = v.rem(j);
            mr = max(mr, rj);
            run = run || rj == rem;
            cnt++;
            if (j + 1 >= hi_i || v.key(j + 1) != kn) break;
            if (cnt == RS_TG) { run = true; break; }
            j++;
        }
        mrn = mr;
    }
    if (edge || run) { want_cand = true; return; }
    const uint32_t lp = has_prev ? min(min(rs_key_lcp(kp, key, a.b, a.key_bits), rem), mrp) : 0u;
    const uint32_t ln = has_next ? min(min(rs_key_lcp(key, kn, a.b, a.key_bits), rem), mrn) : 0u;
    const uint32_t g = max(lp, ln) + 1;
    if (g >= a.g_min || rem <= 64) rs_update(a, rs_col_of_rem(a, rem), g);
}


static inline int rs_layout(const KeyGeom &g) { return g.packed ? FBG_SLOTS_PACKED : g.wide ? FBG_SLOTS_WIDE : FBG_SLOTS_PAIRS; }

static inline void rs_args_init(fbg_ctx *ctx, RankArgs &a, uint64_t *keys, uint32_t *vals, uint64_t slots, int layout, int pb, int b,
                         int key_bits, int K)
{
    a.keys = keys; a.vals = vals; a.T = ctx->text.as<uint8_t>();
    a.pb = layout != FBG_SLOTS_PAIRS ? pb : 0; a.pmask = layout != FBG_SLOTS_PAIRS ? (1ull << pb) - 1 : 0;
    a.N = slots; a.Ntext = ctx->N; a.n = ctx->n; a.row_len = (uint32_t)(ctx->n + 1);
    a.own_lo = 0; a.own_hi = slots; a.first_part = a.last_part = 1; a.part_mode = 0; a.values_only = 0;
    a.magic32 = (uint32_t)((1ull << 32) / (ctx->n + 1));
    a.magic64 = ~0ull / (ctx->n + 1);
    a.b = b; a.key_bits = key_bits; a.K = K; a.reversed = ctx->reversed;
    a.gmax = ctx->gmax.as<uint32_t>();
    a.cand = nullptr; a.pm = nullptr; a.blk_count = nullptr; a.region = 0;
    a.ties = nullptr; a.tie_count = nullptr; a.tie_region = 0; a.pairs = nullptr; a.pair_count = nullptr;
    a.big = ctx->big_groups.as<uint32_t>();
    a.counters = ctx->scalars.as<unsigned long long>() + 32;
    a.g_min = 0;
}

static inline void rs_remember(fbg_ctx *ctx, uint64_t *keys, uint32_t *vals, const KeyGeom &g)
{
    ctx->rk_keys = keys; ctx->sa_ptr = vals;
    ctx->rk_layout = rs_layout(g); ctx->rk_pb = g.pb;
    ctx->rk_b = g.b; ctx->rk_key_bits = g.key_bits; ctx->rk_K = g.K;
}
```

### founderblockgraphs_amd/csrc/rank_scan.hip

```cpp
#include <algorithm>
#include <cstring>
#include <vector>
#include "fbg_internal.h"
#include "text_cmp.h"
#include <rocprim/rocprim.hpp>

#include "rank_common.h"

#define RS_ITEMS 4
#define RS_THREADS 256
#define RS_CHUNK (RS_THREADS * RS_ITEMS)

template <int L, bool PLAIN> __global__ __launch_bounds__(RS_THREADS) __attribute__((amdgpu_waves_per_eu(7, 8))) void k_rank_scan(RankArgs a)
{
    __shared__ uint64_t skey[RS_CHUNK + 2 * RS_HALO];
    __shared__ uint32_t srem[RS_CHUNK + 2 * RS_HALO];
    __shared__ uint16_t sq[RS_CHUNK];
    __shared__ uint32_t sqn, s_cand_n, s_tie_n;
    const int lane = threadIdx.x & 63;
    const uint64_t nchunks = (a.own_hi - a.own_lo + RS_CHUNK - 1) / RS_CHUNK;
    if (threadIdx.x == 0) { s_cand_n = 0; s_tie_n = 0; }
    uint64_t w[RS_ITEMS + 1];
    uint32_t v[RS_ITEMS + 1];
    const int my_i = RS_HALO + RS_ITEMS * (int)threadIdx.x;
// ... 31 lines not shown
            if (my_i + r < hi_i) {
                key = w[r] >> a.pb;
                rem = rs_rem<L>(a, rs_pos_of<L>(a, w[r], v[r]));
            }
            kk[r + 3] = key; cc[r + 2] = rem;
            skey[my_i + r] = key; srem[my_i + r] = rem;
        }
        if (threadIdx.x < 2 * RS_HALO) {
            uint64_t key = 0;
            uint32_t rem = 0;
            if (halo_i >= lo_i && halo_i < hi_i) {
                key = w[RS_ITEMS] >> a.pb;
                rem = rs_rem<L>(a, rs_pos_of<L>(a, w[RS_ITEMS], v[RS_ITEMS]));
            }
            skey[halo_i] = key; srem[halo_i] = rem;
        }
        __syncthreads();
        if (c + gridDim.x < nchunks) fetch(c + gridDim.x);
#pragma unroll
        for (int j = 0; j < 3; j++) {
            kk[j] = __shfl_up(kk[RS_ITEMS + j], 1, 64);
            kk[RS_ITEMS + 3 + j] = __shfl_down(kk[3 + j], 1, 64);
        }
#pragma unroll
        for (int j = 0; j < 2; j++) {
            cc[j] = __shfl_up(cc[RS_ITEMS + j], 1, 64);
            cc[RS_ITEMS + 2 + j] = __shfl_down(cc[2 + j], 1, 64);
        }
        if (lane == 0) {
#pragma unroll
            for (int j = 0; j < 3; j++) kk[j] = skey[my_i - 3 + j];
            cc[0] = srem[my_i - 2]; cc[1] = srem[my_i - 1];
        }
        if (lane == 63) {
#pragma unroll
            for (int j = 0; j < 3; j++) kk[RS_ITEMS + 3 + j] = skey[my_i + RS_ITEMS + j];
            cc[RS_ITEMS + 2] = srem[my_i + RS_ITEMS]; cc[RS_ITEMS + 3] = srem[my_i + RS_ITEMS + 1];
        }
        uint32_t upd_g[RS_ITEMS], upd_c[RS_ITEMS];
#pragma unroll
        for (int r = 0; r < RS_ITEMS; r++) { upd_g[r] = 0; upd_c[r] = 0; }
        uint32_t slow4 = 0, tie4 = 0, cand4 = 0;
        uint32_t lcp[RS_ITEMS + 1];
#pragma unroll
        for (int r = 0; r <= RS_ITEMS; r++) lcp[r] = PLAIN ? rs_key_lcp(kk[r + 2], kk[r + 3], a.b, a.key_bits) : 0u;
#pragma unroll
        for (int r = 0; r < RS_ITEMS; r++) {
            const int i = my_i + r;
            const bool in = i < hi_i;
            const bool window = i - 3 >= lo_i && i + 3 < hi_i;
            const uint64_t key = kk[r + 3];
            const uint32_t rem = cc[r + 2];
            const bool eqp = kk[r + 2] == key, eqn = kk[r + 4] == key;
            bool slow = in && !window;
            bool want_cand = false, want_cand2 = false, want_tie = false;
            if (window) {
                const bool prev_tie = kk[r + 1] == kk[r + 2], next_tie = kk[r + 5] == kk[r + 4];
                if (!eqp && !eqn) {
                    if (rem != 0) {
                        if ((prev_tie && kk[r] == kk[r + 1]) || (next_tie && kk[r + 6] == kk[r + 5])) slow = true;
                        else {
                            bool run = cc[r + 1] == rem || cc[r + 3] == rem;
                            uint32_t mrp = cc[r + 1], mrn = cc[r + 3];
                            if (prev_tie) { run = run || cc[r] == rem; mrp = max(mrp, cc[r]); }
                            if (next_tie) { run = run || cc[r + 4] == rem; mrn = max(mrn, cc[r + 4]); }
                            if (run) want_cand = true;
                            else if (PLAIN) {
                                const uint32_t g = max(min(lcp[r], min(rem, mrp)), min(lcp[r + 1], min(rem, mrn))) + 1;
                                if (g >= a.g_min || rem <= 64) { upd_g[r] = g; upd_c[r] = rs_col_of_rem(a, rem); }
                            } else if (rem <= 64) slow = true;
                        }
                    }
                } else if (!eqp && kk[r + 5] != key && i + 4 < hi_i) {
                    const uint32_t r1 = cc[r + 3], rb = cc[r + 1], ra = cc[r + 4];
                    const bool simple = rem >= (uint32_t)a.K && r1 >= (uint32_t)a.K && rem != r1 &&
                                        !prev_tie && rb != rem && rb != r1 &&
                                        kk[r + 6] != kk[r + 5] && ra != rem && ra != r1;
                    if (simple) want_tie = true;
                    else { want_cand = true; want_cand2 = true; }
                } else if (!(eqp && !eqn && kk[r + 1] != key && i - 4 >= lo_i)) slow = true;
            }
            slow4 |= (slow ? 1u : 0u) << r;
            tie4 |= (want_tie ? 1u : 0u) << r;
            cand4 |= ((want_cand ? 1u : 0u) << r) | ((want_cand2 ? 16u : 0u) << r);
        }
        for (uint32_t bits = slow4; __ballot(bits != 0);) {
            const bool on = bits != 0;
            const int rr = on ? __ffs((int)bits) - 1 : 0;
            bits &= bits - 1;
            const unsigned long long smask = __ballot(on);
            uint32_t qb = 0;
            const int leader = __ffsll((long long)smask) - 1;
            if (lane == leader) qb = atomicAdd(&sqn, (uint32_t)__popcll(smask));
            qb = __shfl(qb, leader, 64);
            if (on) sq[qb + (uint32_t)__popcll(smask & ((1ull << lane) - 1))] = (uint16_t)(my_i + rr);
        }
        if (!a.values_only) {
            const uint32_t k_first = (uint32_t)(base + (uint64_t)(my_i - RS_HALO));
            for (uint32_t bits = tie4; __ballot(bits != 0);) {
                const bool on = bits != 0;
                const int rr = on ? __ffs((int)bits) - 1 : 0;
                bits &= bits - 1;
                rs_append(on, &s_tie_n, a.ties, a.tie_region, k_first + (uint32_t)rr);
            }
            for (uint32_t bits = cand4; __ballot(bits != 0);) {
                const bool on = bits != 0;
                const int rr = on ? __ffs((int)bits) - 1 : 0;
                bits &= bits - 1;
                rs_append(on, &s_cand_n, a.cand, a.region, k_first + (uint32_t)(rr & 3) + (uint32_t)(rr >> 2));
            }
        }
        uint32_t cur[RS_ITEMS];
#pragma unroll
        for (int r = 0; r < RS_ITEMS; r++) cur[r] = (PLAIN && upd_g[r]) ? a.gmax[upd_c[r]] : 0xffffffffu;
        __syncthreads();
        {
            const uint32_t qn = sqn;
            for (uint32_t q0 = 0; q0 < qn; q0 += RS_THREADS) {
                if (q0 + (threadIdx.x & ~63u) >= qn) break;
                const uint32_t q = q0 + threadIdx.x;
                bool want_cand = false, want_tie = false;
                uint64_t k = 0;
                if (q < qn) {
                    const int i = sq[q];
                    k = base + (uint64_t)(i - RS_HALO);
                    const bool is_tie = (i > lo_i && skey[i - 1] == skey[i]) || (i + 1 < hi_i && skey[i + 1] == skey[i]);
                    if (!(a.values_only && is_tie)) rank_scan_slow(a, RsLdsView{skey, srem}, i, lo_i, hi_i, k, want_cand, want_tie);
                }
                if (!a.values_only) {
                    rs_append(want_cand, &s_cand_n, a.cand, a.region, (uint32_t)k);
                    rs_append(want_tie, &s_tie_n, a.ties, a.tie_region, (uint32_t)k);
                }
            }
        }
        if (PLAIN) {
#pragma unroll
            for (int r = 0; r < RS_ITEMS; r++)
                if (cur[r] < upd_g[r]) atomicMax(&a.gmax[upd_c[r]], upd_g[r]);
        }
        __syncthreads();
    }
    if (threadIdx.x == 0 && !a.values_only) { a.blk_count[blockIdx.x] = s_cand_n; a.tie_count[blockIdx.x] = s_tie_n; }
}

#define RL_EV_LO 3
#define RL_EV_HI 60
#define RL_EV (RL_EV_HI - RL_EV_LO + 1)
#define RL_THREADS 256
#define RL_WAVES (RL_THREADS / 64)
#define RL_LIST 128

struct LeanArgs {
    const uint64_t *keys;
    uint64_t own_lo, own_hi;
    uint32_t per_wave, pmask;
    int pb;
    float inv_row_len, eps, one_minus_eps, near_end;
};

__device__ __forceinline__ uint32_t rl_from_next(uint32_t v) { return (uint32_t)__builtin_amdgcn_update_dpp(0, (int)v, 0x130, 0xf, 0xf, false); }
__device__ __forceinline__ uint32_t rl_lanes_below(unsigned long long m)
{
    return __builtin_amdgcn_mbcnt_hi((uint32_t)(m >> 32), __builtin_amdgcn_mbcnt_lo((uint32_t)m, 0u));
}

__device__ __attribute__((noinline)) void rl_noted(const RankArgs &a, const uint2 *list, uint32_t n, uint32_t *s_pair_n)
{
    const int lane = threadIdx.x & 63;
    uint32_t base = 0;
    if (lane == 0) base = atomicAdd(s_pair_n, n);
    base = __shfl(base, 0, 64);
    if ((uint32_t)lane < n && base + (uint32_t)lane < a.tie_region) a.pairs[(size_t)blockIdx.x * a.tie_region + base + lane] = list[lane];
}

__device__ __attribute__((noinline)) void rl_queued(const RankArgs &a, const uint32_t *list, uint32_t n, uint32_t *s_cand_n, uint32_t *s_tie_n)
{
    const int lane = threadIdx.x & 63;
    bool want_cand = false, want_tie = false;
    uint64_t k = 0;
    if ((uint32_t)lane < n) {
        k = list[lane];
        const int64_t base = (int64_t)k - RS_HALO;
        const int lo_i = (int)max((int64_t)0, (int64_t)a.own_lo - base);
        const int hi_i = (int)min((int64_t)(2 * RS_HALO + 1), (int64_t)a.own_hi - base);
        const RsWordView view{a.keys + base, &a, lo_i, hi_i};
        rank_scan_slow(a, view, RS_HALO, lo_i, hi_i, k, want_cand, want_tie);
    }
    rs_append(want_cand, s_cand_n, a.cand, a.region, (uint32_t)k);
    rs_append(want_tie, s_tie_n, a.ties, a.tie_region, (uint32_t)k);
}

template <class E> __device__ __forceinline__ void rl_shift(E *list, uint32_t &n)
{
    const int lane = threadIdx.x & 63;
    const uint32_t rest = n - 64;
    if ((uint32_t)lane < rest) { const E v = list[64 + lane]; list[lane] = v; }
    n = rest;
}

__global__ __launch_bounds__(RL_THREADS) __attribute__((amdgpu_waves_per_eu(8, 8))) void k_rank_scan_lean(const RankArgs *__restrict__ ap, LeanArgs f)
{
    __shared__ uint2 s_note[RL_WAVES][RL_LIST];
    __shared__ uint32_t s_queue[RL_WAVES][RL_LIST];
    __shared__ uint32_t s_cand_n, s_tie_n, s_pair_n;
    const int lane = threadIdx.x & 63;
    const int wv = __builtin_amdgcn_readfirstlane((int)(threadIdx.x >> 6));
    if (threadIdx.x == 0) { s_cand_n = 0; s_tie_n = 0; s_pair_n = 0; }
    __syncthreads();
    uint2 *my_note = s_note[wv];
    uint32_t *my_queue = s_queue[wv];
    uint32_t nn = 0, nq = 0;
    const uint32_t own_lo = (uint32_t)f.own_lo, own_hi = (uint32_t)f.own_hi;
    const uint32_t wlo = own_lo + ((uint32_t)blockIdx.x * RL_WAVES + (uint32_t)wv) * f.per_wave;
    const uint32_t whi = min(own_hi, wlo + f.per_wave);
    const unsigned long long EVM = ((1ull << (RL_EV_HI + 1)) - 1) & ~((1ull << RL_EV_LO) - 1);
    const unsigned long long RNG = ~(1ull << 63);
    const uint64_t *__restrict__ keys = f.keys;
    auto load_row = [&](uint32_t k0) -> uint64_t {
        const uint32_t k = min(max(k0 - RL_EV_LO + (uint32_t)lane, own_lo), own_hi - 1);
        return keys[k];
    };
    uint64_t xnext = wlo < whi ? load_row(wlo) : 0ull;
    for (uint32_t k0 = wlo; k0 < whi; k0 += RL_EV) {
        const uint64_t x = xnext;
        if (k0 + RL_EV < whi) xnext = load_row(k0 + RL_EV);
        const uint32_t slot = k0 - RL_EV_LO + (uint32_t)lane;
        if (k0 < own_lo + 2 * RS_HALO || k0 + RL_EV + 2 * RS_HALO > own_hi || k0 + RL_EV > whi) {
            const unsigned long long Q = EVM & __ballot(slot < whi);
            if ((Q >> lane) & 1ull) my_queue[nq + rl_lanes_below(Q)] = slot;
            nq += (uint32_t)__popcll(Q);
        } else {
            const uint32_t hi = (uint32_t)(x >> 32), lo = (uint32_t)x;
            const uint32_t lo_n = rl_from_next(lo);
            const uint32_t dh = hi ^ rl_from_next(hi), dl = (lo ^ lo_n) >> f.pb;
            const float fr = __builtin_amdgcn_fractf((float)(lo & f.pmask) * f.inv_row_len);
            const float f1 = __uint_as_float(rl_from_next(__float_as_uint(fr))), f2 = __uint_as_float(rl_from_next(__float_as_uint(f1)));
            const float d1 = fabsf(fr - f1), d2 = fabsf(fr - f2);
            const unsigned long long E = __ballot((dh | dl) == 0);
            const unsigned long long R1 = __ballot(d1 < f.eps) | __ballot(d1 > f.one_minus_eps);
            const unsigned long long R2 = __ballot(d2 < f.eps) | __ballot(d2 > f.one_minus_eps);
            const unsigned long long NE = __ballot(fr >= f.near_end) | __ballot(fr < f.eps);
            unsigned long long SS, Q;
            if (((R1 | R2 | NE | (E & (E << 1))) & RNG) == 0) {
                SS = EVM & E & ~((E << 2) | (E >> 2));
                Q = EVM & E & ~SS;
                Q |= Q << 1;
            } else {
                const unsigned long long TIE = E | (E << 1);
                const unsigned long long PH = E & ~((E << 1) | (E >> 1));
                const unsigned long long LONG = TIE & ~(PH | (PH << 1));
                const unsigned long long ADJL = ((LONG >> 1) | (LONG << 1)) & ~TIE;
                SS = EVM & PH & ~(NE | (NE >> 1) | R1 | (R1 << 1) | (R2 << 1) | R2 | (R1 >> 1) | (E << 2) | (E >> 2));
                const unsigned long long QP = EVM & PH & ~SS;
                const unsigned long long RUN = R1 | (R1 << 1) | ((PH & R2) << 2) | ((PH >> 1) & R2);
                Q = QP | (QP << 1) | (EVM & (LONG | ADJL | (~TIE & (RUN | NE))));
            }
            if (SS) {
                if ((SS >> lane) & 1ull) my_note[nn + rl_lanes_below(SS)] = make_uint2(lo & f.pmask, lo_n & f.pmask);
                nn += (uint32_t)__popcll(SS);
            }
            if (Q) {
                if ((Q >> lane) & 1ull) my_queue[nq + rl_lanes_below(Q)] = slot;
                nq += (uint32_t)__popcll(Q);
            }
        }
        while (nq >= 64) { rl_queued(*ap, my_queue, 64, &s_cand_n, &s_tie_n); rl_shift(my_queue, nq); }
        if (nn >= 64) { rl_noted(*ap, my_note, 64, &s_pair_n); rl_shift(my_note, nn); }
    }
    if (nn) rl_noted(*ap, my_note, nn, &s_pair_n);
    if (nq) rl_queued(*ap, my_queue, nq, &s_cand_n, &s_tie_n);
    __syncthreads();
    if (threadIdx.x == 0) { ap->blk_count[blockIdx.x] = s_cand_n; ap->tie_count[blockIdx.x] = s_tie_n; ap->pair_count[blockIdx.x] = s_pair_n; }
}

static bool rs_lean_setup(const RankArgs &a, int pb, unsigned blocks, LeanArgs *f)
{
    const uint64_t own = a.own_hi - a.own_lo, waves = (uint64_t)blocks * RL_WAVES;
    f->per_wave = (uint32_t)(((own + waves - 1) / waves + RL_EV - 1) / RL_EV * RL_EV);
    f->keys = a.keys; f->own_lo = a.own_lo; f->own_hi = a.own_hi; f->pmask = (uint32_t)a.pmask; f->pb = pb;
    const double L = (double)a.row_len;
    const double delta = (ldexp(1.0, pb - 25) + ldexp(1.0, pb - 22) + 2.0) / L + 1e-6;
    f->inv_row_len = (float)(1.0 / L);
    f->eps = (float)(2.0 * delta);
    f->one_minus_eps = 1.0f - f->eps;
    f->near_end = (float)(1.0 - 65.0 / L - delta);
    return 2.0 * delta < 0.01 && pb <= 31 && a.own_hi < (1ull << 31);
}

template <int L> __global__ __launch_bounds__(256) void k_tie_simple(RankArgs a)
{
    const uint32_t have = a.tie_count[blockIdx.x];
    if (have > a.tie_region) { if (threadIdx.x == 0) a.counters[1] = 1; return; }
    for (uint32_t e = threadIdx.x; e < have; e += blockDim.x) {
        const uint64_t h = a.ties[(size_t)blockIdx.x * a.tie_region + e];
        uint64_t key[RS_TG], pos[RS_TG];
        uint32_t best[RS_TG];
#pragma unroll
        for (int i = 0; i < RS_TG; i++) {
            const bool ok = h + i < a.own_hi;
            const uint64_t w = ok ? a.keys[h + i] : 0ull;
            key[i] = w >> a.pb;
            pos[i] = rs_pos_of<L>(a, w, (ok && L != FBG_SLOTS_PACKED) ? a.vals[h + i] : 0u);
            if (!ok) key[i] = ~key[0];
            best[i] = 0;
        }
        int s = 1;
#pragma unroll
        for (int i = 1; i < RS_TG; i++)
            if (s == i && key[i] == key[0]) s = i + 1;
        const uint64_t x01 = fbg_load8(a.T, pos[0] + a.K) ^ fbg_load8(a.T, pos[1] + a.K);
#pragma unroll
        for (int i = 0; i < RS_TG; i++)
#pragma unroll
            for (int j = i + 1; j < RS_TG; j++)
                if (j < s) {
                    uint32_t x;
                    if (i == 0 && j == 1 && x01 != 0) x = (uint32_t)(__ffsll((unsigned long long)x01) - 1) / 8;
                    else x = fbg_extend_match(a.T, pos[i] + a.K, pos[j] + a.K, 0);
                    best[i] = max(best[i], x);
                    best[j] = max(best[j], x);
                }
#pragma unroll
        for (int i = 0; i < RS_TG; i++)
            if (i < s) rs_update(a, rs_col_of_rem(a, rs_rem<L>(a, pos[i])), fbg_clamp_lcp(best[i] + (uint32_t)a.K) + 1);
    }
}

__global__ __launch_bounds__(256) void k_tie_pairs(RankArgs a)
{
    const uint32_t have = a.pair_count[blockIdx.x];
    if (have > a.tie_region) { if (threadIdx.x == 0) a.counters[1] = 1; return; }
    for (uint32_t e = threadIdx.x; e < have; e += blockDim.x) {
        const uint2 p = a.pairs[(size_t)blockIdx.x * a.tie_region + e];
        const uint64_t x = fbg_load8(a.T, (uint64_t)p.x + a.K) ^ fbg_load8(a.T, (uint64_t)p.y + a.K);
        const uint32_t h = x != 0 ? (uint32_t)(__ffsll((unsigned long long)x) - 1) / 8 : fbg_extend_match(a.T, (uint64_t)p.x + a.K, (uint64_t)p.y + a.K, 8);
        const uint32_t g = fbg_clamp_lcp(h + (uint32_t)a.K) + 1;
        rs_update(a, rs_col_of_rem(a, rs_rem<FBG_SLOTS_PACKED>(a, p.x)), g);
        rs_update(a, rs_col_of_rem(a, rs_rem<FBG_SLOTS_PACKED>(a, p.y)), g);
    }
}

__global__ __launch_bounds__(256) void k_tie_sample(const uint64_t *__restrict__ keys, int shift, uint64_t N, int b, int key_bits,
                                                    unsigned long long *__restrict__ counters,
                                                    unsigned int *__restrict__ hist)
{
    __shared__ unsigned int sh[64];
    __shared__ unsigned int sties;
    if (threadIdx.x < 64) sh[threadIdx.x] = 0;
    if (threadIdx.x == 0) sties = 0;
    __syncthreads();
    const uint64_t k = (uint64_t)blockIdx.x * 1024 * 256 + threadIdx.x;
    uint32_t bin = 0xffffffffu;
    if (k < N) {
        const uint64_t key = keys[k] >> shift;
        const uint64_t kp = k > 0 ? keys[k - 1] >> shift : ~key, kn = k + 1 < N ? keys[k + 1] >> shift : ~key;
        if (kp == key || kn == key) {
            bin = 64;
        } else {
            const uint32_t lp = k > 0 ? rs_key_lcp(kp, key, b, key_bits) : 0u;
            const uint32_t ln = k + 1 < N ? rs_key_lcp(key, kn, b, key_bits) : 0u;
            bin = min(max(lp, ln) + 1, 63u);
        }
    }
    {
        const int lane = threadIdx.x & 63;
        unsigned long long rest = __ballot(bin != 0xffffffffu);
        while (rest) {
            const int l = __ffsll((long long)rest) - 1;
            const uint32_t v = __shfl(bin, l, 64);
            const unsigned long long same = __ballot(bin == v);
            if (lane == l) { if (v == 64) atomicAdd(&sties, (uint32_t)__popcll(same)); else atomicAdd(&sh[v], (uint32_t)__popcll(same)); }
            rest &= ~same;
        }
    }
    __syncthreads();
    if (threadIdx.x < 64 && sh[threadIdx.x]) atomicAdd(&hist[threadIdx.x], sh[threadIdx.x]);
    if (threadIdx.x == 0) {
        atomicAdd(&counters[2], (unsigned long long)sties);
        atomicAdd(&counters[3], (unsigned long long)min((uint64_t)256, N - (uint64_t)blockIdx.x * 1024 * 256));
    }
}

__global__ void k_count_unfilled(const uint32_t *__restrict__ gmax, uint64_t n, uint32_t g_min, int reversed,
                                 unsigned long long *__restrict__ counters)
{
    const uint64_t x = (uint64_t)blockIdx.x * blockDim.x + threadIdx.x;
    const uint64_t rem = reversed ? x + 1 : n - x;
    const bool miss = x < n && rem > 64 && gmax[x] < g_min;
    const unsigned long long mask = __ballot(miss);
    if ((threadIdx.x & 63) == 0 && mask) atomicAdd(&counters[1 + 3], (unsigned long long)__popcll(mask));
}

__global__ void k_cand_compact(const uint32_t *__restrict__ regions, const uint32_t *__restrict__ counts,
                               const uint32_t *__restrict__ offsets, uint32_t region, uint32_t *__restrict__ out)
{
    const uint32_t c = counts[blockIdx.x] < region ? counts[blockIdx.x] : region, o = offsets[blockIdx.x];
    for (uint32_t i = threadIdx.x; i < c; i += blockDim.x) out[o + i] = regions[(size_t)blockIdx.x * region + i];
}

#define RS_BIG_GROUPS 1024
#define RS_BIG_MEMBERS 8192
template <int L> __global__ void k_tie_groups(RankArgs a, uint64_t T, int by_list)
{
    const uint64_t t = (uint64_t)blockIdx.x * blockDim.x + threadIdx.x;
    if (t >= T) return;
    const uint64_t k0 = by_list ? (uint64_t)a.cand[t] : a.own_lo + t;
    const uint64_t key = rs_key<L>(a, k0);
    if (k0 > a.own_lo && rs_key<L>(a, k0 - 1) == key) return;
    if (k0 + 1 >= a.own_hi || rs_key<L>(a, k0 + 1) != key) return;
    uint32_t s = 1;
    while (k0 + s < a.own_hi && s <= RS_BIG_MEMBERS && rs_key<L>(a, k0 + s) == key) s++;
    if (s > 64) {
        if (s > RS_BIG_MEMBERS) { a.counters[1] = 1; return; }
        const unsigned long long e = atomicAdd(&a.counters[5], 1ull);
        if (e >= RS_BIG_GROUPS) { a.counters[1] = 1; return; }
        a.big[2 * e] = (uint32_t)k0;
        a.big[2 * e + 1] = s;
        return;
    }
    typedef typename PosT<L>::type pos_t;
    pos_t pos[64];
    uint32_t from = (uint32_t)a.K;
    for (uint32_t i = 0; i < s; i++) {
        pos[i] = (pos_t)rs_pos<L>(a, k0 + i);
        if (rs_rem<L>(a, pos[i]) < (uint32_t)a.K) from = 0;
    }
    for (uint32_t i = 1; i < s; i++) {
        const pos_t cur = pos[i];
        uint32_t j = i;
        while (j > 0) {
            const pos_t o = pos[j - 1];
            const uint32_t h = fbg_extend_match(a.T, (uint64_t)o + from, (uint64_t)cur + from, 0);
            if (a.T[(uint64_t)o + from + h] < a.T[(uint64_t)cur + from + h]) break;
            pos[j] = o;
            j--;
        }
        pos[j] = cur;
    }
    for (uint32_t i = 0; i < s; i++) rs_set_pos<L>(a, k0 + i, pos[i]);
}

template <int L> __global__ __launch_bounds__(256) void k_tie_big(RankArgs a, int exact)
{
    __shared__ uint32_t pos_lo[RS_BIG_MEMBERS];
    __shared__ uint8_t pos_hi[L == FBG_SLOTS_WIDE ? RS_BIG_MEMBERS : 1];
    __shared__ uint8_t cls[RS_BIG_MEMBERS];
    __shared__ uint32_t offs[66];
    __shared__ uint32_t q_start, q_count;
    if (blockIdx.x >= a.counters[5]) return;
    const uint64_t k0 = a.big[2 * blockIdx.x];
    const uint32_t s = a.big[2 * blockIdx.x + 1];
    auto member = [&](uint32_t i) -> uint64_t {
        return L == FBG_SLOTS_WIDE ? ((uint64_t)pos_hi[L == FBG_SLOTS_WIDE ? i : 0] << 32) | pos_lo[i] : (uint64_t)pos_lo[i];
    };
    if (threadIdx.x < 66) offs[threadIdx.x] = 0;
    __syncthreads();
    for (uint32_t i = threadIdx.x; i < s; i += blockDim.x) {
        const uint64_t p = rs_pos<L>(a, k0 + i);
        const uint32_t c = min(rs_rem<L>(a, p), (uint32_t)a.K);
        pos_lo[i] = (uint32_t)p;
        if (L == FBG_SLOTS_WIDE) pos_hi[L == FBG_SLOTS_WIDE ? i : 0] = (uint8_t)(p >> 32);
        cls[i] = (uint8_t)c;
        atomicAdd(&offs[c + 1], 1u);
    }
    __syncthreads();
    if (threadIdx.x == 0) {
        q_count = offs[a.K + 1];
        for (int c = 1; c <= a.K + 1; c++) offs[c] += offs[c - 1];
        q_start = offs[a.K];
    }
    __syncthreads();
    if (!exact) {
        for (uint32_t i = threadIdx.x; i < s; i += blockDim.x) {
            const uint32_t dst = atomicAdd(&offs[cls[i]], 1u);
            rs_set_pos<L>(a, k0 + dst, member(i));
        }
        __threadfence();
        __syncthreads();
        if (threadIdx.x == 0) {
            const uint32_t q = q_count;
            if (q > 64) { a.counters[1] = 1; return; }
            const uint64_t kq = k0 + q_start;
            for (uint32_t i = 1; i < q; i++) {
                const uint64_t cur = rs_pos<L>(a, kq + i);
                uint32_t j = i;
                while (j > 0) {
                    const uint64_t o = rs_pos<L>(a, kq + j - 1);
                    const uint32_t h = fbg_extend_match(a.T, o + a.K, cur + a.K, 0);
                    if (a.T[o + a.K + h] < a.T[cur + a.K + h]) break;
                    rs_set_pos<L>(a, kq + j, o);
                    j--;
// ... 36 lines not shown
    pr[p] = rs_slot_lcp<L>(a, k + 1);
}

template <int L> __global__ void k_runs(RankArgs a, uint64_t T)
{
    const uint64_t t = (uint64_t)blockIdx.x * blockDim.x + threadIdx.x;
    if (t >= T) return;
    const uint64_t k0 = a.cand[t];
    const uint32_t col = rs_col<L>(a, k0);
    if (col == a.n) return;
    if (k0 > a.own_lo && rs_col<L>(a, k0 - 1) == col) return;
    const uint64_t lo_slot = a.first_part ? a.own_lo : 0, hi_slot = a.last_part ? a.own_hi : a.N;
    uint64_t ks = k0;
    while (ks > lo_slot && rs_col<L>(a, ks - 1) == col) ks--;
    if (ks == 0 && !a.first_part) { a.counters[1] = 1; return; }
    uint32_t run = rs_slot_lcp<L>(a, ks);
    uint64_t s = ks;
    for (;;) {
        if (s >= k0 && s < a.own_hi) a.pm[t + (s - k0)] = run;
        if (s + 1 >= hi_slot || rs_col<L>(a, s + 1) != col) break;
        s++;
        run = min(run, rs_slot_lcp<L>(a, s));
    }
    if (s + 1 == a.N && !a.last_part) { a.counters[1] = 1; return; }
    uint32_t rmin = 0xffffffffu;
    for (;; s--) {
        rmin = min(rmin, rs_slot_lcp<L>(a, s + 1));
        if (s >= k0 && s < a.own_hi) rs_update(a, col, max(a.pm[t + (s - k0)], rmin) + 1);
        if (s == ks || s <= k0) break;
    }
}

struct FinishArgs {
    const uint32_t *gmax;
    uint64_t n, x0, x1;
    int mode, disable_tricks;
    uint64_t *out;
};

__global__ void k_rank_finish(FinishArgs a)
{
    const uint64_t x = a.x0 + (uint64_t)blockIdx.x * blockDim.x + threadIdx.x;
    if (x >= a.x1) return;
    const unsigned long long g = a.gmax[x];
    if (a.mode == FBG_SCAN_V) {
        a.out[x] = g <= x + 1 ? x + 1 - g : x + 1;
        return;
    }
    unsigned long long fx = x;
    const bool any_active = a.disable_tricks || x != 0;
    if (any_active && g > 0) {
        const unsigned long long gg = x + g;
        const unsigned long long fi = gg > a.n ? (a.disable_tricks ? a.n : a.n - 1) : gg - 1;
        fx = max(fx, fi);
    }
    a.out[x] = max((unsigned long long)a.out[x], fx);
}

template <class F> static int rs_with_tmp(fbg_ctx *ctx, F &&call)
{
    size_t bytes = 0;
    hipError_t e = call(nullptr, bytes);
    if (e != hipSuccess) return fbg_fail(ctx, FBG_ERR_HIP, "rocprim size query: %s", hipGetErrorString(e));
    FBG_TRY(fbg_reserve(ctx, ctx->tmp, bytes));
    size_t have = ctx->tmp.cap;
    e = call(ctx->tmp.p, have);
    if (e != hipSuccess) return fbg_fail(ctx, FBG_ERR_HIP, "rocprim call: %s", hipGetErrorString(e));
    return FBG_OK;
}

#define RS_LAUNCH(kernel, layout, grid, block, st, ...)                                                     \
    do {                                                                                                    \
        if ((layout) == FBG_SLOTS_PACKED) hipLaunchKernelGGL((kernel<FBG_SLOTS_PACKED>), grid, block, 0, st, __VA_ARGS__);  \
        else if ((layout) == FBG_SLOTS_WIDE) hipLaunchKernelGGL((kernel<FBG_SLOTS_WIDE>), grid, block, 0, st, __VA_ARGS__); \
        else hipLaunchKernelGGL((kernel<FBG_SLOTS_PAIRS>), grid, block, 0, st, __VA_ARGS__);                                \
    } while (0)

#define RS_LAUNCH_SCAN(layout, plain, grid, st, args)                                                                         \
    do {                                                                                                                     \
        const dim3 blk_(RS_THREADS);                                                                                         \
        if ((layout) == FBG_SLOTS_PACKED) { if (plain) hipLaunchKernelGGL((k_rank_scan<FBG_SLOTS_PACKED, true>), grid, blk_, 0, st, args);   \
                                            else hipLaunchKernelGGL((k_rank_scan<FBG_SLOTS_PACKED, false>), grid, blk_, 0, st, args); }      \
        else if ((layout) == FBG_SLOTS_WIDE) { if (plain) hipLaunchKernelGGL((k_rank_scan<FBG_SLOTS_WIDE, true>), grid, blk_, 0, st, args);  \
                                               else hipLaunchKernelGGL((k_rank_scan<FBG_SLOTS_WIDE, false>), grid, blk_, 0, st, args); }     \
        else { if (plain) hipLaunchKernelGGL((k_rank_scan<FBG_SLOTS_PAIRS, true>), grid, blk_, 0, st, args);                               \
               else hipLaunchKernelGGL((k_rank_scan<FBG_SLOTS_PAIRS, false>), grid, blk_, 0, st, args); }                                  \
    } while (0)

static int rs_fork(fbg_ctx *ctx)
{
    if (!ctx->aux) {
        FBG_HIP_TRY(ctx, hipStreamCreateWithFlags(&ctx->aux, hipStreamNonBlocking));
        FBG_HIP_TRY(ctx, hipEventCreateWithFlags(&ctx->aux_fork, hipEventDisableTiming));
        FBG_HIP_TRY(ctx, hipEventCreateWithFlags(&ctx->aux_join, hipEventDisableTiming));
    }
    FBG_HIP_TRY(ctx, hipEventRecord(ctx->aux_fork, ctx->stream));
    FBG_HIP_TRY(ctx, hipStreamWaitEvent(ctx->aux, ctx->aux_fork, 0));
    ctx->aux_pending = true;
    return FBG_OK;
}
static int rs_join(fbg_ctx *ctx)
{
    if (!ctx->aux_pending) return FBG_OK;
    ctx->aux_pending = false;
    FBG_HIP_TRY(ctx, hipEventRecord(ctx->aux_join, ctx->aux));
    FBG_HIP_TRY(ctx, hipStreamWaitEvent(ctx->stream, ctx->aux_join, 0));
    return FBG_OK;
}

static int rs_order_candidates(fbg_ctx *ctx, RankArgs &a, int layout, uint64_t T, int *launches)
{
    hipStream_t st = ctx->stream;
    FBG_TRY(fbg_reserve(ctx, ctx->dp_a, T * 4));
    FBG_TRY(fbg_reserve(ctx, ctx->dp_b, T * 4));
    uint32_t *sorted = ctx->dp_a.as<uint32_t>();
    uint32_t *flat = ctx->dp_e.as<uint32_t>();
    FBG_TRY(rs_with_tmp(ctx, [&](void *tmp, size_t &bytes) {
        return rocprim::radix_sort_keys(tmp, bytes, flat, sorted, (size_t)T, 0u, 32u, st);
    }));
    a.cand = sorted;
    a.pm = ctx->dp_b.as<uint32_t>();
    RS_LAUNCH(k_tie_groups, layout, dim3(fbg_blocks(T, 64)), dim3(64), st, a, T, 1);
    RS_LAUNCH(k_tie_big, layout, dim3(RS_BIG_GROUPS), dim3(256), st, a, 0);
    *launches += 3;
    return FBG_OK;
}

static int rs_classify(fbg_ctx *ctx, RankArgs &a, int layout, uint64_t *T_out, int *launches)
{
    hipStream_t st = ctx->stream;
    const uint64_t own = a.own_hi - a.own_lo;
    const unsigned rs_blocks = fbg_blocks(own, RS_CHUNK, 256 * 16);
    const uint32_t region = (uint32_t)((own / rs_blocks) / 8 + 256);
    const uint32_t tie_region = (uint32_t)((own / rs_blocks) / 6 + 256);
    FBG_TRY(fbg_reserve(ctx, ctx->list, (size_t)rs_blocks * region * 4));
    FBG_TRY(fbg_reserve(ctx, ctx->tie_list, (size_t)rs_blocks * tie_region * 4));
    FBG_TRY(fbg_reserve(ctx, ctx->big_groups, RS_BIG_GROUPS * 8));
    a.big = ctx->big_groups.as<uint32_t>();
    FBG_TRY(fbg_reserve(ctx, ctx->dp_c, (size_t)(rs_blocks + 1) * 4));
    FBG_TRY(fbg_reserve(ctx, ctx->dp_d, (size_t)(rs_blocks + 1) * 4));
    FBG_TRY(fbg_reserve(ctx, ctx->dp_f, (size_t)(rs_blocks + 1) * 4));
    FBG_HIP_TRY(ctx, hipMemsetAsync(ctx->dp_c.p, 0, (size_t)(rs_blocks + 1) * 4, st));
    FBG_HIP_TRY(ctx, hipMemsetAsync(ctx->dp_f.p, 0, (size_t)(rs_blocks + 1) * 4, st));
    a.cand = ctx->list.as<uint32_t>();
    a.blk_count = ctx->dp_c.as<uint32_t>(); a.region = region;
    a.ties = ctx->tie_list.as<uint32_t>();
    a.tie_count = ctx->dp_f.as<uint32_t>(); a.tie_region = tie_region;
    FBG_TRY(fbg_stage_begin(ctx, FBG_STAGE_RANK_KERNEL));
    LeanArgs lf;
    const bool lean = layout == FBG_SLOTS_PACKED && a.g_min > (uint32_t)a.K && !a.values_only && !a.part_mode && !ctx->opt.rank_no_lean &&
                      rs_lean_setup(a, a.pb, rs_blocks, &lf);
    if (lean)
    {
        FBG_TRY(fbg_reserve(ctx, ctx->ps_g, (size_t)rs_blocks * tie_region * 8));
        FBG_TRY(fbg_reserve(ctx, ctx->ps_h, (size_t)rs_blocks * 4));
        a.pairs = ctx->ps_g.as<uint2>(); a.pair_count = ctx->ps_h.as<uint32_t>();
        static_assert(sizeof(RankArgs) <= sizeof(ctx->kargs_host), "room for the scan's arguments");
        FBG_TRY(fbg_reserve(ctx, ctx->kargs, sizeof(RankArgs)));
        memcpy(ctx->kargs_host, &a, sizeof(RankArgs));
        FBG_HIP_TRY(ctx, hipMemcpyAsync(ctx->kargs.p, ctx->kargs_host, sizeof(RankArgs), hipMemcpyHostToDevice, st));
        hipLaunchKernelGGL(k_rank_scan_lean, dim3(rs_blocks), dim3(RL_THREADS), 0, st, (const RankArgs *)ctx->kargs.p, lf);
    }
    else
        RS_LAUNCH_SCAN(layout, a.g_min <= (uint32_t)a.K || a.values_only, dim3(rs_blocks), st, a);
    FBG_TRY(fbg_stage_end(ctx, FBG_STAGE_RANK_KERNEL, 1));
    {
        hipStream_t ts = st;
        if (!ctx->opt.no_aux_stream) { FBG_TRY(rs_fork(ctx)); ts = ctx->aux; }
        if (lean) hipLaunchKernelGGL(k_tie_pairs, dim3(rs_blocks), dim3(256), 0, ts, a);
        RS_LAUNCH(k_tie_simple, layout, dim3(rs_blocks), dim3(256), ts, a);
    }
    *launches += 2;
    const int rc_rest = [&]() -> int {
        uint32_t *d_counts = a.blk_count, *d_offs = ctx->dp_d.as<uint32_t>();
        FBG_TRY(rs_with_tmp(ctx, [&](void *tmp, size_t &bytes) {
            return rocprim::exclusive_scan(tmp, bytes, d_counts, d_offs, 0u, (size_t)(rs_blocks + 1), rocprim::plus<uint32_t>(), st);
        }));
        uint32_t *d_max = reinterpret_cast<uint32_t *>(a.counters + 6);
        FBG_TRY(rs_with_tmp(ctx, [&](void *tmp, size_t &bytes) {
            return rocprim::reduce(tmp, bytes, d_counts, d_max, 0u, (size_t)rs_blocks, rocprim::maximum<uint32_t>(), st);
        }));
        uint32_t tot = 0, mx = 0;
        FBG_HIP_TRY(ctx, hipMemcpyAsync(&tot, d_offs + rs_blocks, 4, hipMemcpyDeviceToHost, st));
        FBG_HIP_TRY(ctx, hipMemcpyAsync(&mx, d_max, 4, hipMemcpyDeviceToHost, st));
        FBG_HIP_TRY(ctx, hipStreamSynchronize(st));
        const uint64_t T = tot;
        *T_out = T;
        if (mx > region) { *T_out = ~0ull; return rs_join(ctx); }
        if (T > 0) {
            FBG_TRY(fbg_reserve(ctx, ctx->dp_e, T * 4));
            uint32_t *flat = ctx->dp_e.as<uint32_t>();
            hipLaunchKernelGGL(k_cand_compact, dim3(rs_blocks), dim3(256), 0, st, a.cand, d_counts, d_offs, region, flat);
            FBG_TRY(rs_order_candidates(ctx, a, layout, T, launches));
        }
        return FBG_OK;
    }();
    if (rc_rest != FBG_OK) { (void)rs_join(ctx); return rc_rest; }
    return FBG_OK;
}

static int rs_pick_threshold(fbg_ctx *ctx, RankArgs &a, const uint64_t *keys, uint64_t count, const KeyGeom &geom, int *reject,
                             int *launches)
{
    *reject = 0;
    if (count <= (1u << 22)) return FBG_OK;
    hipStream_t st = ctx->stream;
    unsigned long long *cnt = a.counters;
    unsigned int *d_hist = reinterpret_cast<unsigned int *>(cnt + 8);
    FBG_HIP_TRY(ctx, hipMemsetAsync(d_hist, 0, 64 * sizeof(unsigned int), st));
    hipLaunchKernelGGL(k_tie_sample, dim3(fbg_blocks(count, 1024 * 256)), dim3(256), 0, st, keys, a.pb, count, geom.b, geom.key_bits,
                       cnt, d_hist);
    (*launches)++;
    unsigned long long hs[4];
    unsigned int hh[64];
    FBG_HIP_TRY(ctx, hipMemcpyAsync(hs, cnt, sizeof(hs), hipMemcpyDeviceToHost, st));
    FBG_HIP_TRY(ctx, hipMemcpyAsync(hh, d_hist, sizeof(hh), hipMemcpyDeviceToHost, st));
    FBG_HIP_TRY(ctx, hipStreamSynchronize(st));
    if (hs[2] * 4 > hs[3]) { *reject = 1; return FBG_OK; }
    if (!ctx->opt.rank_no_threshold) {
        const double need = 32.0 / (double)ctx->m * (double)hs[3];
        unsigned long long above = 0;
        for (int g = 63; g >= 1; g--) {
            above += hh[g];
            if ((double)above >= need) { a.g_min = (uint32_t)g; break; }
        }
        if ((double)hs[2] / (double)hs[3] * (double)ctx->m >= 32.0) a.g_min = (uint32_t)geom.K + 1;
    }
    return FBG_OK;
}

int fbg_rank_scan_try(fbg_ctx *ctx, uint64_t *keys, uint32_t *vals, const KeyGeom &geom, int *done)
{
    *done = 0;
    ctx->ranked = false;
    ctx->part_active = false;
    const uint64_t N = ctx->N, n = ctx->n;
    const int layout = rs_layout(geom);
    hipStream_t st = ctx->stream;
    FBG_TRY(fbg_stage_begin(ctx, FBG_STAGE_RANKSCAN));
    unsigned long long *cnt = ctx->scalars.as<unsigned long long>() + 32;
    int launches = 0;
    FBG_TRY(fbg_reserve(ctx, ctx->gmax, (n + 1) * 4));
    RankArgs a;
    rs_args_init(ctx, a, keys, vals, N, layout, geom.pb, geom.b, geom.key_bits, geom.K);
    uint64_t T = 0;
    FBG_HIP_TRY(ctx, hipMemsetAsync(cnt, 0, 8 * sizeof(unsigned long long), st));
    FBG_HIP_TRY(ctx, hipMemsetAsync(ctx->gmax.p, 0, (n + 1) * 4, st));
    int reject = 0;
    FBG_TRY(rs_pick_threshold(ctx, a, keys, N, geom, &reject, &launches));
    if (reject) return fbg_stage_end(ctx, FBG_STAGE_RANKSCAN, launches);
    FBG_TRY(rs_classify(ctx, a, layout, &T, &launches));
    if (T == ~0ull) return fbg_stage_end(ctx, FBG_STAGE_RANKSCAN, launches);
    if (T > 0) {
        RS_LAUNCH(k_runs, layout, dim3(fbg_blocks(T, 64)), dim3(64), st, a, T);
        launches++;
    }
    FBG_TRY(rs_join(ctx));
    unsigned long long h[5];
    if (a.g_min > 1)
        hipLaunchKernelGGL(k_count_unfilled, dim3(fbg_blocks(n, 256)), dim3(256), 0, st, a.gmax, n, a.g_min, a.reversed, cnt);
    FBG_HIP_TRY(ctx, hipMemcpyAsync(h, cnt, sizeof(h), hipMemcpyDeviceToHost, st));
    FBG_HIP_TRY(ctx, hipStreamSynchronize(st));
    launches++;
    if (h[1] != 0) return fbg_stage_end(ctx, FBG_STAGE_RANKSCAN, launches);
    if (a.g_min > 1 && h[4] != 0) {
        a.g_min = 0;
        a.values_only = 1;
        RS_LAUNCH_SCAN(layout, true, dim3(fbg_blocks(N, RS_CHUNK, 256 * 16)), st, a);
        launches++;
    }
    FBG_HIP_TRY(ctx, hipGetLastError());
    ctx->n_exc = 0;
    ctx->ranked = true;
    rs_remember(ctx, keys, vals, geom);
    *done = 1;
    return fbg_stage_end(ctx, FBG_STAGE_RANKSCAN, launches);
}

__global__ void k_halo_export(const uint64_t *__restrict__ keys, const uint32_t *__restrict__ vals, uint64_t own_lo,
                              uint64_t own_hi, uint64_t ok, uint8_t *__restrict__ blob)
{
    uint64_t *bk = reinterpret_cast<uint64_t *>(blob);
    uint32_t *bv = reinterpret_cast<uint32_t *>(blob + 2 * FBG_PART_HALO * 8);
    uint64_t *tail = reinterpret_cast<uint64_t *>(blob + 2 * FBG_PART_HALO * 12);
    const uint32_t t = threadIdx.x;
    if (ok & 1) {
        const uint64_t k = t < FBG_PART_HALO ? own_lo + t : own_hi - 2 * FBG_PART_HALO + t;
        bk[t] = keys[k]; bv[t] = vals ? vals[k] : 0u;
    } else { bk[t] = 0; bv[t] = 0; }
    if (t == 0) { tail[0] = ok; tail[1] = own_hi - own_lo; }
}

__global__ void k_halo_import(const uint8_t *__restrict__ blobs, int part, int nparts, uint64_t own_lo, uint64_t own_hi,
                              uint64_t *__restrict__ keys, uint32_t *__restrict__ vals)
{
    const uint32_t t = threadIdx.x;
    if (part > 0) {
        const uint8_t *bl = blobs + (size_t)(part - 1) * FBG_PART_HALO_BYTES;
        keys[t] = reinterpret_cast<const uint64_t *>(bl)[FBG_PART_HALO + t];
        if (vals) vals[t] = reinterpret_cast<const uint32_t *>(bl + 2 * FBG_PART_HALO * 8)[FBG_PART_HALO + t];
    }
    if (part + 1 < nparts) {
        const uint8_t *bl = blobs + (size_t)(part + 1) * FBG_PART_HALO_BYTES;
        keys[own_hi + t] = reinterpret_cast<const uint64_t *>(bl)[t];
        if (vals) vals[own_hi + t] = reinterpret_cast<const uint32_t *>(bl + 2 * FBG_PART_HALO * 8)[t];
    }
}

static void rs_part_args(fbg_ctx *ctx, RankArgs &a)
{
    rs_args_init(ctx, a, ctx->rk_keys, ctx->sa_ptr, ctx->part_count + 2 * FBG_PART_HALO, ctx->rk_layout, ctx->rk_pb, ctx->rk_b,
                 ctx->rk_key_bits, ctx->rk_K);
    a.own_lo = FBG_PART_HALO; a.own_hi = FBG_PART_HALO + ctx->part_count;
    a.first_part = ctx->part == 0; a.last_part = ctx->part + 1 == ctx->nparts;
    a.part_mode = ctx->nparts > 1;
}

int fbg_rank_part_classify(fbg_ctx *ctx, uint64_t *keys, uint32_t *vals, uint64_t count, const KeyGeom &geom, int pre_ok,
                           uint8_t *d_blob, int *ok)
{
    const uint64_t n = ctx->n;
    hipStream_t st = ctx->stream;
    FBG_TRY(fbg_stage_begin(ctx, FBG_STAGE_RANKSCAN));
    int launches = 0;
    ctx->ranked = false;
    ctx->part_count = count;
    ctx->part_T = 0;
    rs_remember(ctx, keys, vals, geom);
    const int layout = rs_layout(geom);
    FBG_TRY(fbg_reserve(ctx, ctx->gmax, (n + 1) * 4));
    unsigned long long *cnt = ctx->scalars.as<unsigned long long>() + 32;
    FBG_HIP_TRY(ctx, hipMemsetAsync(cnt, 0, 8 * sizeof(unsigned long long), st));
    FBG_HIP_TRY(ctx, hipMemsetAsync(ctx->gmax.p, 0, (n + 1) * 4, st));
    int good = pre_ok && count >= 2 * FBG_PART_HALO;
    RankArgs a;
    rs_part_args(ctx, a);
    if (good) {
        int reject = 0;
        FBG_TRY(rs_pick_threshold(ctx, a, keys + a.own_lo, count, geom, &reject, &launches));
        if (reject) good = 0;
    }
    ctx->part_gmin = a.g_min;
    if (good) {
        uint64_t T = 0;
        FBG_TRY(rs_classify(ctx, a, layout, &T, &launches));
        FBG_TRY(rs_join(ctx));
        if (T == ~0ull) good = 0;
        else {
            ctx->part_T = T;
            unsigned long long h[2];
            FBG_HIP_TRY(ctx, hipMemcpyAsync(h, cnt, sizeof(h), hipMemcpyDeviceToHost, st));
            FBG_HIP_TRY(ctx, hipStreamSynchronize(st));
            if (h[1] != 0) good = 0;
        }
    }
    hipLaunchKernelGGL(k_halo_export, dim3(1), dim3(2 * FBG_PART_HALO), 0, st, keys, vals, a.own_lo, a.own_hi,
                       (uint64_t)good | ((uint64_t)a.g_min << 8), d_blob);
    launches++;
    FBG_HIP_TRY(ctx, hipGetLastError());
    *ok = good;
    return fbg_stage_end(ctx, FBG_STAGE_RANKSCAN, launches);
}

int fbg_rank_part_runs(fbg_ctx *ctx, const uint8_t *d_blobs, uint32_t *d_gmax, int *ok)
{
    const uint64_t n = ctx->n;
    hipStream_t st = ctx->stream;
    FBG_TRY(fbg_stage_begin(ctx, FBG_STAGE_RANKSCAN));
    int launches = 0;
    std::vector<uint8_t> hb((size_t)ctx->nparts * FBG_PART_HALO_BYTES);
    FBG_HIP_TRY(ctx, hipMemcpyAsync(hb.data(), d_blobs, hb.size(), hipMemcpyDeviceToHost, st));
    FBG_HIP_TRY(ctx, hipStreamSynchronize(st));
    int good = 1;
    uint32_t gmin_all = 0;
    for (int p = 0; p < ctx->nparts; p++) {
        uint64_t tail[2];
        memcpy(tail, hb.data() + (size_t)p * FBG_PART_HALO_BYTES + 2 * FBG_PART_HALO * 12, sizeof(tail));
        if (!(tail[0] & 1)) good = 0;
        gmin_all = std::max(gmin_all, (uint32_t)(tail[0] >> 8));
    }
    ctx->part_gmin = gmin_all;
    if (good) {
        RankArgs a;
        rs_part_args(ctx, a);
        a.cand = ctx->dp_a.as<uint32_t>(); a.pm = ctx->dp_b.as<uint32_t>();
        hipLaunchKernelGGL(k_halo_import, dim3(1), dim3(FBG_PART_HALO), 0, st, d_blobs, ctx->part, ctx->nparts, a.own_lo,
                           a.own_hi, a.keys, a.vals);
        launches++;
        if (ctx->part_T > 0) {
            RS_LAUNCH(k_runs, ctx->rk_layout, dim3(fbg_blocks(ctx->part_T, 64)), dim3(64), st, a, ctx->part_T);
            launches++;
            unsigned long long h[2];
            FBG_HIP_TRY(ctx, hipMemcpyAsync(h, a.counters, sizeof(h), hipMemcpyDeviceToHost, st));
            FBG_HIP_TRY(ctx, hipStreamSynchronize(st));
            if (h[1] != 0) good = 0;
        }
    }
    FBG_HIP_TRY(ctx, hipMemcpyAsync(d_gmax, ctx->gmax.p, (n + 1) * 4, hipMemcpyDeviceToDevice, st));
    const uint32_t verdict = good ? 0u : 1u;
    FBG_HIP_TRY(ctx, hipMemcpyAsync(d_gmax + n, &verdict, 4, hipMemcpyHostToDevice, st));
    FBG_HIP_TRY(ctx, hipStreamSynchronize(st));
    *ok = good;
    return fbg_stage_end(ctx, FBG_STAGE_RANKSCAN, launches);
}

int fbg_rank_part_unfilled(fbg_ctx *ctx, uint64_t *unfilled)
{
    *unfilled = 0;
    if (ctx->part_gmin <= 1) return FBG_OK;
    hipStream_t st = ctx->stream;
    unsigned long long *cnt = ctx->scalars.as<unsigned long long>() + 32;
    FBG_HIP_TRY(ctx, hipMemsetAsync(cnt + 4, 0, sizeof(unsigned long long), st));
    hipLaunchKernelGGL(k_count_unfilled, dim3(fbg_blocks(ctx->n, 256)), dim3(256), 0, st, ctx->gmax.as<uint32_t>(), ctx->n, ctx->part_gmin,
                       ctx->reversed, cnt);
    unsigned long long h = 0;
// ... 43 lines not shown
```

### founderblockgraphs_amd/csrc/suffix_sort.hip

```cpp
#include "fbg_internal.h"
#include "text_cmp.h"
#include <rocprim/rocprim.hpp>
#include <utility>
#include <cmath>

#define SS_THREADS 256

using fbg_sort_config = rocprim::radix_sort_config<
    rocprim::default_config, rocprim::default_config,
    rocprim::radix_sort_onesweep_config<rocprim::kernel_config<512, 32>, rocprim::kernel_config<1024, 8>, 9,
                                        rocprim::block_radix_rank_algorithm::match>>;

#define PK_ITEMS 8
#define FBG_SEP 0x80
struct PackArgs {
    const uint8_t *T;
    uint64_t N;
    const uint8_t *code;
    int b, K, pb;
    uint64_t *keys;
    uint32_t *vals;
    uint64_t lo, hi, cap;
    int nohi;
    unsigned long long *counter;
// ... 565 lines not shown
    vals_new[k] = vals_old[s];
    grp_new[k] = grp_old[s];
}

__global__ void k_doubling_keys(const uint32_t *__restrict__ vals, const uint32_t *__restrict__ grp, uint64_t cnt,
                                const uint4 *__restrict__ rec, uint64_t h, uint64_t N, int nb,
                                uint64_t *__restrict__ keys)
{
    uint64_t k = (uint64_t)blockIdx.x * blockDim.x + threadIdx.x;
    if (k >= cnt) return;
    uint64_t q = (uint64_t)vals[k] + h;
    uint32_t r2 = q < N ? rec[q].x : 0u;
    keys[k] = ((uint64_t)grp[k] << nb) | r2;
}

__global__ void k_iota(uint32_t *__restrict__ a, uint64_t cnt)
{
    uint64_t k = (uint64_t)blockIdx.x * blockDim.x + threadIdx.x;
    if (k < cnt) a[k] = (uint32_t)k;
}

static int ensure_tmp(fbg_ctx *ctx, size_t bytes) { return fbg_reserve(ctx, ctx->tmp, bytes); }

template <class F> static int with_tmp(fbg_ctx *ctx, F &&call)
{
    size_t bytes = 0;
    hipError_t e = call(nullptr, bytes);
    if (e != hipSuccess) return fbg_fail(ctx, FBG_ERR_HIP, "rocprim size query: %s", hipGetErrorString(e));
    FBG_TRY(ensure_tmp(ctx, bytes));
    size_t have = ctx->tmp.cap;
    e = call(ctx->tmp.p, have);
    if (e != hipSuccess)
        return fbg_fail(ctx, e == hipErrorOutOfMemory ? FBG_ERR_OOM : FBG_ERR_HIP, "rocprim call: %s", hipGetErrorString(e));
    return FBG_OK;
}

int fbg_key_setup(fbg_ctx *ctx, bool compact, KeyGeom *g, int *launches)
{
    const uint64_t N = ctx->N;
    hipStream_t st = ctx->stream;
    uint8_t *d_code = ctx->small.as<uint8_t>() + 2048;
    const uint64_t *hist = ctx->byte_hist;
    if (hist[0] != 1)
        return fbg_fail(ctx, FBG_ERR_INVALID, "the MSA contains a NUL byte; the text needs a unique 0 sentinel");
    int below = 0, real = 0;
    for (int c = 1; c < 256; c++)
        if (hist[c] && c != '#') { real++; if (c < '#') below++; }
    compact = compact && below == 0 && real >= 1 && real < FBG_SEP;
    uint8_t code[256];
    int sigma = 0;
    if (compact) {
        for (int c = 0; c < 256; c++) {
            if (c == 0 || c == '#') { code[c] = FBG_SEP; continue; }
            code[c] = (uint8_t)sigma;
            if (hist[c]) sigma++;
        }
    } else {
        for (int c = 0; c < 256; c++) { code[c] = (uint8_t)sigma; if (hist[c]) sigma++; }
    }
    int b = 1;
    while ((1 << b) < sigma) b++;
    double H = 0;
    for (int c = 1; c < 256; c++)
        if (hist[c] && !(compact && c == '#')) { const double q = (double)hist[c] / (double)N; H -= q * log2(q); }
    if (H < 0.05) H = 0.05;
    int K = (int)ceil((log2((double)N) + 5.0) / H);
    if (ctx->opt.full_keys || K > 64 / b) K = 64 / b;
    {
        const int passes = (K * b + 8) / 9;
        const int Kfill = (9 * passes) / b;
        K = Kfill < 64 / b ? Kfill : 64 / b;
    }
    g->compact = compact; g->packed = false; g->wide = false; g->pb = 0;
    if (N >= (1ull << 32) || (compact && ctx->opt.force_wide)) {
        if (!compact) return fbg_fail(ctx, FBG_ERR_TOO_LARGE, "text length %llu needs >32-bit positions", (unsigned long long)N);
        int pb = 1;
        while ((1ull << (32 + pb)) < N) pb++;
        g->wide = true; g->pb = pb;
        if (K > (64 - pb) / b) K = (64 - pb) / b;
    } else if (compact && !ctx->opt.no_packed) {
        int pb = 1;
        while ((1ull << pb) < N) pb++;
        const int Kroom = (64 - pb) / b;
        const int Kmin = (int)ceil((log2((double)N) + 3.2) / H);
        if (Kroom >= Kmin) { g->packed = true; g->pb = pb; if (K > Kroom) K = Kroom; }
    }
    g->b = b; g->K = K; g->key_bits = K * b; g->d_code = d_code;
    FBG_HIP_TRY(ctx, hipMemcpyAsync(d_code, code, 256, hipMemcpyHostToDevice, st));
    FBG_HIP_TRY(ctx, hipStreamSynchronize(st));
    *launches += 1;
    return FBG_OK;
}

static int sort_slots(fbg_ctx *ctx, const KeyGeom &g, uint64_t count, uint64_t out_offset)
{
    hipStream_t st = ctx->stream;
    uint64_t *ka = ctx->keysA.as<uint64_t>(), *kb = ctx->keysB.as<uint64_t>() + out_offset;
    if (g.packed) {
        unsigned lo = (unsigned)g.pb;
        const unsigned hi = (unsigned)(g.pb + g.key_bits);
        if (hi == 64 && count < (1u << 23)) lo = 0;
        return with_tmp(ctx, [&](void *tmp, size_t &bytes) {
            return rocprim::radix_sort_keys<fbg_sort_config>(tmp, bytes, ka, kb, (size_t)count, lo, hi, st);
        });
    }
    uint32_t *va = ctx->valsA.as<uint32_t>(), *vb = ctx->valsB.as<uint32_t>() + out_offset;
    unsigned lo = g.wide ? (unsigned)g.pb : ctx->sp_key_flags ? 2u : 0u;
    const unsigned hi = lo + (unsigned)g.key_bits;
    if (hi == 64 && count < (1u << 23)) lo = 0;
    return with_tmp(ctx, [&](void *tmp, size_t &bytes) {
        return rocprim::radix_sort_pairs<fbg_sort_config>(tmp, bytes, ka, kb, va, vb, (size_t)count, lo, hi, st);
    });
}

static int sample_says_similar(fbg_ctx *ctx, const KeyGeom &g, bool *similar, int *launches)
{
    const uint64_t N = ctx->N;
    hipStream_t st = ctx->stream;
    *similar = false;
    if (N < (1u << 22)) return FBG_OK;
    const uint64_t S = 1u << 20, stride = N / S;
    FBG_TRY(fbg_reserve(ctx, ctx->dp_g, S * 8));
    FBG_TRY(fbg_reserve(ctx, ctx->dp_h, S * 8));
    uint64_t *smp = ctx->dp_g.as<uint64_t>(), *srt = ctx->dp_h.as<uint64_t>();
    unsigned long long *d_count = ctx->scalars.as<unsigned long long>() + 8;
    FBG_HIP_TRY(ctx, hipMemsetAsync(d_count, 0, 8, st));
    hipLaunchKernelGGL(k_sample_keys, dim3(fbg_blocks(S, 256)), dim3(256), 0, st, ctx->text.as<uint8_t>(), N, g.d_code, g.b, g.K,
                       g.compact ? 1 : 0, stride, S, smp);
    FBG_TRY(with_tmp(ctx, [&](void *tmp, size_t &bytes) {
        return rocprim::radix_sort_keys(tmp, bytes, smp, srt, (size_t)S, 0u, (unsigned)g.key_bits, st);
    }));
    hipLaunchKernelGGL(k_count_equal_neighbours, dim3(fbg_blocks(S, 256)), dim3(256), 0, st, srt, S, d_count);
    unsigned long long twins = 0;
    FBG_HIP_TRY(ctx, hipMemcpyAsync(&twins, d_count, 8, hipMemcpyDeviceToHost, st));
    FBG_HIP_TRY(ctx, hipStreamSynchronize(st));
    *launches += 3;
    const double est = (double)twins * (double)N / ((double)S * (double)S);
    *similar = est > 0.5;
    return FBG_OK;
}

int fbg_suffix_sort(fbg_ctx *ctx)
{
    const uint64_t N = ctx->N;
    hipStream_t st = ctx->stream;
    FBG_TRY(fbg_stage_begin(ctx, FBG_STAGE_SUFFIX_SORT));
    int launches = 0;
    const uint8_t *T = ctx->text.as<uint8_t>();
    ctx->part_active = false;
    ctx->ranked = false;
    ctx->granked = false;
    ctx->grs_ebits = nullptr;
    ctx->grs_flagged = false;
    KeyGeom g;

    if (ctx->gapfree && !ctx->have_ignore && !ctx->opt.no_ranked) {
        if (!fbg_msd_pre_geom(ctx, &g)) FBG_TRY(fbg_key_setup(ctx, true, &g, &launches));
        bool similar = false;
        FBG_TRY(sample_says_similar(ctx, g, &similar, &launches));
        uint64_t *sorted = nullptr;
        int msd_ok = 0;
        FBG_TRY(fbg_msd_sort(ctx, g, &sorted, &msd_ok, &launches));
        if (!msd_ok) {
            FBG_TRY(fbg_reserve(ctx, ctx->keysA, N * 8));
            FBG_TRY(fbg_reserve(ctx, ctx->keysB, N * 8));
            if (!g.packed) {
                FBG_TRY(fbg_reserve(ctx, ctx->valsA, N * 4));
                FBG_TRY(fbg_reserve(ctx, ctx->valsB, N * 4));
            }
            PackArgs pa;
            pa.T = T; pa.N = N; pa.code = g.d_code; pa.b = g.b; pa.K = g.K; pa.pb = g.pb;
            pa.keys = ctx->keysA.as<uint64_t>(); pa.vals = ctx->valsA.as<uint32_t>();
            pa.lo = pa.hi = pa.cap = 0; pa.nohi = 1; pa.counter = nullptr;
            launch_pack(ctx, g, false, pa);
            launches++;
            FBG_TRY(sort_slots(ctx, g, N, 0));
            sorted = ctx->keysB.as<uint64_t>();
        }
        uint32_t *svals = g.packed ? nullptr : ctx->valsB.as<uint32_t>();
        int done = 0;
        if (!similar && ctx->opt.pure_scan != 1) FBG_TRY(fbg_rank_scan_try(ctx, sorted, svals, g, &done));
        if (!done && ctx->opt.pure_scan != -1) FBG_TRY(fbg_pure_scan_try(ctx, sorted, svals, g, &done));
        if (done) {
            FBG_HIP_TRY(ctx, hipGetLastError());
            return fbg_stage_end(ctx, FBG_STAGE_SUFFIX_SORT, launches);
        }
    }

    FBG_TRY(fbg_key_setup(ctx, false, &g, &launches));
    int b = g.b, K = g.K, key_bits = g.key_bits;
    FBG_TRY(fbg_reserve(ctx, ctx->keysA, N * 8));
    FBG_TRY(fbg_reserve(ctx, ctx->keysB, N * 8));
    FBG_TRY(fbg_reserve(ctx, ctx->valsA, N * 4));
    FBG_TRY(fbg_reserve(ctx, ctx->valsB, N * 4));
    uint64_t *keysA = ctx->keysA.as<uint64_t>(), *keysB = ctx->keysB.as<uint64_t>();
    uint32_t *valsA = ctx->valsA.as<uint32_t>(), *valsB = ctx->valsB.as<uint32_t>();
    uint32_t *grp = nullptr;
    uint4 *rec = nullptr;
    uint8_t *flags = nullptr;
    uint32_t *sa = valsB;
    ctx->sa_ptr = sa;
    ColTest ct;
    ct.colT = ctx->gapfree ? nullptr : ctx->colT.as<uint32_t>();
    ct.row_len = (uint32_t)(ctx->n + 1);
    ct.n = (uint32_t)ctx->n;
    ct.last = (uint32_t)(N - 1);
    ctx->pairs_similar = false;
    ctx->spanned = false;
    ctx->sort_payload = nullptr;
    ctx->sp_key_flags = false;
    bool try_span = fbg_span_eligible(ctx, g);
    if (try_span && ctx->opt.span_scan != 1 && ctx->opt.span_scan != 3) {
        bool similar = false;
        FBG_TRY(sample_says_similar(ctx, g, &similar, &launches));
        try_span = similar;
    }
    const bool try_grs = !try_span && (!ctx->gapfree || ctx->have_ignore) && !ctx->reversed && !ctx->grs_skip && ctx->opt.gapped_rank != -1 && K <= 32;
    if (try_grs || try_span) FBG_TRY(fbg_grs_prepare(ctx, &launches));
    if (try_span) {
        ctx->grs_ebits = nullptr; ctx->grs_flagged = false;
        ctx->sp_key_flags = fbg_span_key_flags(ctx, g);
        K = g.K; key_bits = g.key_bits;
        FBG_TRY(fbg_span_prepare(ctx, g, &launches));
        ctx->sort_payload = ctx->sp_cells.as<uint32_t>();
    }
    {
        int ss_ok = 0;
        FBG_TRY(fbg_sample_sort_pairs(ctx, g, &ss_ok, &launches));
        if (!ss_ok) {
            PackArgs pa;
            pa.T = T; pa.N = N; pa.code = g.d_code; pa.b = b; pa.K = K; pa.pb = 0;
            pa.keys = ctx->keysA.as<uint64_t>(); pa.vals = ctx->valsA.as<uint32_t>();
            pa.lo = pa.hi = pa.cap = 0; pa.nohi = 1; pa.counter = nullptr;
            pa.ebits = ctx->grs_ebits;
            pa.payload = ctx->sort_payload;
            pa.key_flags = ctx->sp_key_flags ? ctx->sp_flagT.as<uint8_t>() : nullptr;
            launch_pack(ctx, g, false, pa);
            launches++;
            FBG_TRY(sort_slots(ctx, g, N, 0));
        }
        ctx->sort_payload = nullptr;
        ctx->sp_key_flags_sorted = ctx->sp_key_flags;
        ctx->sp_key_flags = false;
        keysA = ctx->keysA.as<uint64_t>(); keysB = ctx->keysB.as<uint64_t>();
        valsA = ctx->valsA.as<uint32_t>(); valsB = ctx->valsB.as<uint32_t>();
        sa = valsB;
        ctx->sa_ptr = sa;
    }
    ctx->grs_ebits = nullptr;
    if (try_span) {
        int done = 0;
        FBG_TRY(fbg_span_try(ctx, keysB, valsB, g, &done));
        if (done) {
            FBG_HIP_TRY(ctx, hipGetLastError());
            return fbg_stage_end(ctx, FBG_STAGE_SUFFIX_SORT, launches);
        }
    } else if (try_grs && ctx->pairs_similar) FBG_TRY(fbg_grs_strip(ctx, valsB));
    else if (try_grs) {
        int done = 0;
        FBG_TRY(fbg_grs_try(ctx, keysB, valsB, g, &done));
        if (done) {
            FBG_HIP_TRY(ctx, hipGetLastError());
            return fbg_stage_end(ctx, FBG_STAGE_SUFFIX_SORT, launches);
        }
        FBG_TRY(fbg_grs_strip(ctx, valsB));
    }
    FBG_TRY(fbg_build_cell_tables(ctx));
    FBG_TRY(fbg_reserve(ctx, ctx->grp, N * 4));
    FBG_TRY(fbg_reserve(ctx, ctx->flags, (N + FC_TILE - 1) / FC_TILE * FC_TILE));
    FBG_TRY(fbg_reserve(ctx, ctx->rec, N * 16));
    grp = ctx->grp.as<uint32_t>();
    rec = ctx->rec.as<uint4>();
    flags = ctx->flags.as<uint8_t>();
    hipLaunchKernelGGL(k_mark_heads, dim3(fbg_blocks(N, 256)), dim3(256), 0, st, keysB, N, (const uint32_t *)nullptr, grp);
    FBG_TRY(with_tmp(ctx, [&](void *tmp, size_t &bytes) {
        return rocprim::inclusive_scan(tmp, bytes, grp, grp, (size_t)N, rocprim::maximum<uint32_t>(), st);
    }));
    const uint64_t bp_min = ctx->opt.bp_min >= 0 ? (uint64_t)ctx->opt.bp_min : (1ull << 24);
    const bool by_position = N >= bp_min && N > 2 * BP_LEAF && N <= 1500000000ull && !ctx->opt.record_scatter;
    if (by_position) {
        int bits = 0;
        while ((1ull << bits) < N) bits++;
        const int S = bits - BP_LEAF_BITS, d1 = (S + 1) / 2, d2 = S - d1;
        FBG_TRY(fbg_reserve(ctx, ctx->msd_w, N * 16));
        FBG_TRY(fbg_reserve(ctx, ctx->msd_v, N * 16));
        const uint64_t nleaf = (N + BP_LEAF - 1) >> BP_LEAF_BITS, ntop = (N >> (d2 + BP_LEAF_BITS)) + 1;
        const uint64_t nwin = (N >> BP_WIN_BITS) + 1;
        FBG_TRY(fbg_reserve(ctx, ctx->list, (ntop + nleaf + 2) * 8 + 3 * nwin * 4));
        unsigned long long *cur1 = ctx->list.as<unsigned long long>(), *cur2 = cur1 + ntop + 1;
        uint2 *win = reinterpret_cast<uint2 *>(cur1 + ntop + nleaf + 2);
        uint32_t *win_lo = reinterpret_cast<uint32_t *>(win + nwin);
        if (ct.colT) {
            hipLaunchKernelGGL(k_bp_windows, dim3(fbg_blocks(nwin, 4)), dim3(256), 0, st, ct.colT, N, ct.n, win, win_lo);
            launches++;
        }
        unsigned long long *bflag = ctx->scalars.as<unsigned long long>() + 120;
        FBG_HIP_TRY(ctx, hipMemsetAsync(cur1, 0, (ntop + nleaf + 2) * 8, st));
        FBG_HIP_TRY(ctx, hipMemsetAsync(bflag, 0, 8, st));
        BpArgs a;
        a.N = N; a.flag = bflag;
        a.grp = grp; a.vals = valsB; a.keys = keysB; a.b = b; a.key_bits = key_bits; a.ct = ct; a.flags = flags;
        a.win = win; a.win_lo = win_lo;
        a.shift = d2 + BP_LEAF_BITS; a.nd = 1u << d1; a.in = nullptr; a.seg_shift = 0; a.tiles_per_seg = 0;
        a.out = ctx->msd_w.as<uint4>(); a.cursor = cur1;
        hipLaunchKernelGGL(k_bp_groups0, dim3(fbg_blocks(N, BP_TILE)), dim3(BP_THREADS), 0, st, a);
        a.in = ctx->msd_w.as<uint4>(); a.seg_shift = d2 + BP_LEAF_BITS;
// ... 181 lines not shown
```

Baseline: 59.06 million.

## Extend MSD sort keys with four extra symbols to resolve tie-pair LCPs

With 2-bit codes, the MSD sort now builds its keys over four more symbols. Those extra 8 bits are carried through the passes using tile-local indices and stored in a per-suffix byte array. The rank scan reads these bytes to encode, in spare pair bits, how many of the extra symbols match. k_tie_pairs can then settle most tie pairs without random text loads, and for the rest it starts comparing text 4 symbols later. The cost is an extra N-byte buffer and write, wider sort keys, more bit packing, and a stats memset and copy.

Result: faster. 60.40 million (median of 6 runs) (+2.3%).

```diff
diff --git a/founderblockgraphs_amd/csrc/ctx.hip b/founderblockgraphs_amd/csrc/ctx.hip
--- a/founderblockgraphs_amd/csrc/ctx.hip
+++ b/founderblockgraphs_amd/csrc/ctx.hip
@@ -173,6 +173,7 @@
     {"dp_literal", &FbgOptions::dp_literal}, {"dp_wave", &FbgOptions::dp_wave}, {"dp_safe_window", &FbgOptions::dp_safe_window},
     {"dp_tile", &FbgOptions::dp_tile}, {"pure_scan", &FbgOptions::pure_scan}, {"gapped_rank", &FbgOptions::gapped_rank}, {"part_tricks_off", &FbgOptions::part_tricks_off}, {"msd_sample_bins", &FbgOptions::msd_sample_bins}, {"msd_min_force", &FbgOptions::msd_min_force}, {"msd_probe", &FbgOptions::msd_probe}, {"msd_xcd", &FbgOptions::msd_xcd}, {"rank_no_lean", &FbgOptions::rank_no_lean}, {"no_stream_upload", &FbgOptions::no_stream_upload},
     {"span_scan", &FbgOptions::span_scan}, {"span_key_flags", &FbgOptions::span_key_flags}, {"span_slow_split", &FbgOptions::span_slow_split}, {"poison", &FbgOptions::poison}, {"dpw_matrix", &FbgOptions::dpw_matrix}, {"dp_chain1", &FbgOptions::dp_chain1},
+    {"msd_ext", &FbgOptions::msd_ext},
 };
 
 static void options_from_env(FbgOptions &o)
@@ -207,6 +208,8 @@
     if (strcmp(key, "dp_kind") == 0) { *value = ctx->dp_kind; return FBG_OK; }
     if (strcmp(key, "msd_decline") == 0) { *value = ctx->msd_decline; return FBG_OK; }
     if (strcmp(key, "pass1_ahead") == 0) { *value = ctx->pass1_ahead; return FBG_OK; }
+    if (strcmp(key, "ext_pairs") == 0) { *value = ctx->ext_pairs; return FBG_OK; }
+    if (strcmp(key, "text_pairs") == 0) { *value = ctx->text_pairs; return FBG_OK; }
     if (strcmp(key, "alloc_calls") == 0) { *value = (int64_t)ctx->alloc_calls; return FBG_OK; }
     if (strcmp(key, "alloc_us") == 0) { *value = (int64_t)ctx->alloc_us; return FBG_OK; }
     if (strcmp(key, "span_decline") == 0) { *value = ctx->sp_decline; return FBG_OK; }
@@ -274,7 +277,7 @@
     (void)hipStreamSynchronize(ctx->stream);
     DevBuf *bufs[] = {&ctx->msa_own, &ctx->text, &ctx->pos, &ctx->tot, &ctx->segtab, &ctx->exc_scratch, &ctx->prow, &ctx->igrow, &ctx->rec,
                       &ctx->xlist, &ctx->gmax, &ctx->excol, &ctx->xslot, &ctx->xbits, &ctx->exc, &ctx->colT, &ctx->keysA, &ctx->keysB, &ctx->valsA, &ctx->valsB, &ctx->grp, &ctx->flags,
-                      &ctx->list, &ctx->tie_list, &ctx->big_groups, &ctx->kargs, &ctx->msd_w, &ctx->msd_v, &ctx->tmp, &ctx->small, &ctx->scalars, &ctx->dp_a, &ctx->dp_b, &ctx->dp_c,
+                      &ctx->msd_ext, &ctx->list, &ctx->tie_list, &ctx->big_groups, &ctx->kargs, &ctx->msd_w, &ctx->msd_v, &ctx->tmp, &ctx->small, &ctx->scalars, &ctx->dp_a, &ctx->dp_b, &ctx->dp_c,
                       &ctx->dp_d, &ctx->dp_e, &ctx->dp_f, &ctx->dp_g, &ctx->dp_h, &ctx->io_a, &ctx->io_b,
                       &ctx->io_c, &ctx->io_d, &ctx->bt_up, &ctx->bt_dep, &ctx->ps_a, &ctx->ps_b, &ctx->ps_c, &ctx->ps_d,
                       &ctx->ps_e, &ctx->ps_f, &ctx->ps_g, &ctx->ps_h, &ctx->gwin, &ctx->gbits, &ctx->gwin_rows,
@@ -342,7 +345,7 @@
     FBG_HIP_TRY(ctx, hipSetDevice(ctx->device));
     FBG_HIP_TRY(ctx, hipStreamSynchronize(ctx->stream));
     const bool sorted_in_A = (ctx->ranked || ctx->granked) && ctx->rk_keys == ctx->keysA.as<uint64_t>();
-    DevBuf *bufs[] = {sorted_in_A ? &ctx->keysB : &ctx->keysA, &ctx->valsA, &ctx->grp, &ctx->flags, &ctx->list, &ctx->tie_list, &ctx->msd_w, &ctx->msd_v,
+    DevBuf *bufs[] = {sorted_in_A ? &ctx->keysB : &ctx->keysA, &ctx->valsA, &ctx->grp, &ctx->flags, &ctx->list, &ctx->tie_list, &ctx->msd_w, &ctx->msd_v, &ctx->msd_ext,
                       &ctx->tmp, &ctx->dp_a, &ctx->dp_b, &ctx->dp_c, &ctx->dp_d, &ctx->dp_e, &ctx->dp_f,
                       &ctx->dp_g, &ctx->dp_h, &ctx->ps_a, &ctx->ps_b, &ctx->ps_c, &ctx->ps_d, &ctx->ps_e, &ctx->ps_f,
                       &ctx->ps_g, &ctx->ps_h, &ctx->sp_cells, &ctx->sp_flagT, &ctx->sp_tiles};
diff --git a/founderblockgraphs_amd/csrc/fbg_internal.h b/founderblockgraphs_amd/csrc/fbg_internal.h
--- a/founderblockgraphs_amd/csrc/fbg_internal.h
+++ b/founderblockgraphs_amd/csrc/fbg_internal.h
@@ -32,7 +32,7 @@
     int64_t no_ranked = 0, no_packed = 0, force_wide = 0, full_keys = 0, no_msd_sort = 0, msd_min = -1, bp_min = -1,
             record_scatter = 0, lcp_text = 0, no_aux_stream = 0, rank_no_threshold = 0, dp_literal = 0, dp_wave = 0,
             dp_safe_window = 0, dp_tile = 0, pure_scan = 0, gapped_rank = 0, part_tricks_off = 0, msd_sample_bins = 0, msd_min_force = 0, msd_probe = 0, msd_xcd = -1, rank_no_lean = 0, no_stream_upload = 0,
-            span_scan = 0, span_key_flags = 0, span_slow_split = 0, poison = 0, dpw_matrix = 0, dp_chain1 = 0;
+            span_scan = 0, span_key_flags = 0, span_slow_split = 0, poison = 0, dpw_matrix = 0, dp_chain1 = 0, msd_ext = 1;
 };
 
 struct fbg_ctx {
@@ -59,6 +59,8 @@
     alignas(16) unsigned char pre_state[768];
     uint64_t pre_tiles = 0;
     int pass1_ahead = 0;
+    bool msd_ext_valid = false;
+    int64_t ext_pairs = -1, text_pairs = -1;
 
     bool index_valid = false;
     int reversed = 0;
@@ -126,6 +128,7 @@
     uint32_t part_gmin = 0;
 
     DevBuf keysA, keysB, valsA, valsB, grp, flags, list, tie_list, big_groups, tmp, small, scalars;
+    DevBuf msd_ext;
     DevBuf kargs;
     alignas(16) unsigned char kargs_host[512];
     DevBuf msd_w, msd_v;
diff --git a/founderblockgraphs_amd/csrc/msd_sort.hip b/founderblockgraphs_amd/csrc/msd_sort.hip
--- a/founderblockgraphs_amd/csrc/msd_sort.hip
+++ b/founderblockgraphs_amd/csrc/msd_sort.hip
@@ -8,6 +8,10 @@
 #define MSD_NB (1 << MSD_DIG)
 #define MSD_THREADS 1024
 #define MSD_TILE (MSD_THREADS * MSD_ITEMS)
+#define MSD_TILE_BITS 13
+#define MSD_XSYM 4
+#define MSD_XBITS 8
+static_assert(MSD_TILE == 1 << MSD_TILE_BITS, "tile size");
 #define MSD_FN_THREADS 512
 #define MSD_FN_CAP 4096
 #define MSD_FN_ITEMS (MSD_FN_CAP / MSD_FN_THREADS)
@@ -22,6 +26,8 @@
     uint64_t N;
     const uint8_t *code;
     int b, K, pb, kb;
+    int xb;
+    uint8_t *ext;
     uint64_t *buf1;
     uint64_t cap1;
     int xs;
@@ -62,7 +68,7 @@
     __syncthreads();
 }
 
-template <bool FULL>
+template <bool FULL, bool EXT>
 __device__ __forceinline__ void msd_pack_split_body(const MsdArgs &a, uint64_t *buf, const uint8_t *cd, uint32_t *cnt, uint32_t *loff, uint32_t *gdelta,
                                                     uint32_t *wsum)
 {
@@ -73,21 +79,22 @@
     __syncthreads();
     const int t0 = threadIdx.x * MSD_ITEMS;
     uint64_t w[MSD_ITEMS];
-    msd_build_keys(tile, t0, b, K, w);
+    msd_build_keys(tile, t0, b, EXT ? K + MSD_XSYM : K, w);
     __syncthreads();
     uint32_t rk[MSD_ITEMS];
-    const int dshift = a.kb - MSD_DIG;
+    const int dshift = a.kb + (EXT ? MSD_XBITS : 0) - MSD_DIG;
 #pragma unroll
     for (int i = 0; i < MSD_ITEMS; i++) {
         const uint64_t p = base + t0 + i;
         const bool ok = FULL || p < a.N;
         rk[i] = ok ? atomicAdd(&cnt[(uint32_t)(w[i] >> dshift)], 1u) : 0xffffffffu;
-        w[i] = (w[i] << a.pb) | p;
+        w[i] = EXT ? (w[i] << MSD_TILE_BITS) | (uint64_t)(t0 + i) : (w[i] << a.pb) | p;
     }
     __syncthreads();
     const uint32_t xq = a.xs > 1 ? (blockIdx.x & (uint32_t)(a.xs - 1)) : 0u;
     msd_scan_and_reserve(cnt, loff, gdelta, wsum, a.count1 + (threadIdx.x < MSD_NB ? threadIdx.x * a.xs + xq : 0), true, nullptr);
-    const int wshift = a.pb + dshift;
+    const int wshift = (EXT ? MSD_TILE_BITS : a.pb) + dshift;
+    const uint64_t kmask = (1ull << a.kb) - 1;
     uint64_t *const obase = a.buf1 + xq * a.segcap;
 #pragma unroll
     for (int i = 0; i < MSD_ITEMS; i++)
@@ -99,8 +106,9 @@
     for (int r = 0; r < MSD_ITEMS; r++) {
         const uint32_t j = threadIdx.x + r * MSD_THREADS;
         if (FULL || j < have) {
-            const uint64_t x = buf[j];
+            uint64_t x = buf[j];
             const uint32_t d = (uint32_t)(x >> wshift);
+            if (EXT) x = (((x >> MSD_TILE_BITS) & kmask) << a.pb) | (base + (x & (MSD_TILE - 1)));
             const uint32_t at = j + gdelta[d];
             if (at < a.segcap) obase[(uint64_t)d * a.cap1 + at] = x;
             else over = true;
@@ -109,6 +117,7 @@
     if (over) atomicOr(a.flag, 2ull);
 }
 
+template <bool EXT>
 __global__ __launch_bounds__(MSD_THREADS) void k_msd_pack_split(MsdArgs a)
 {
     __shared__ uint64_t buf[MSD_TILE];
@@ -119,7 +128,13 @@
     if (threadIdx.x < 256) cd[threadIdx.x] = a.code[threadIdx.x];
     if (threadIdx.x < MSD_NB) cnt[threadIdx.x] = 0;
     __syncthreads();
-    msd_pack_split_body<false>(a, buf, cd, cnt, loff, gdelta, wsum);
+    msd_pack_split_body<false, EXT>(a, buf, cd, cnt, loff, gdelta, wsum);
+}
+
+static void msd_launch_pass1(const MsdArgs &a, unsigned tiles, hipStream_t st)
+{
+    if (a.xb) hipLaunchKernelGGL(k_msd_pack_split<true>, dim3(tiles), dim3(MSD_THREADS), 0, st, a);
+    else hipLaunchKernelGGL(k_msd_pack_split<false>, dim3(tiles), dim3(MSD_THREADS), 0, st, a);
 }
 
 __global__ __launch_bounds__(1024) void k_msd_tiles(const unsigned long long *__restrict__ count1, uint64_t segcap, uint32_t nseg,
@@ -159,7 +174,7 @@
 __device__ __forceinline__ void msd_split_body(const MsdArgs &a, uint64_t *buf, uint32_t *cnt, uint32_t *loff, uint32_t *gdelta, uint32_t *wsum,
                                                const uint64_t *__restrict__ in, uint32_t have, uint32_t seg)
 {
-    const int wshift = a.pb + a.kb - 2 * MSD_DIG;
+    const int wshift = a.pb + a.kb - 2 * MSD_DIG + a.xb;
     uint64_t w[MSD_ITEMS];
     uint32_t rk[MSD_ITEMS];
 #pragma unroll
@@ -351,8 +366,8 @@
 }
 
 template <int CAP, int THREADS>
-__device__ __forceinline__ void msd_finish_body(uint64_t *buf, uint32_t *cnt, uint32_t *loff, uint32_t *wsum, const uint64_t *in_a,
-                                                uint32_t n_a, const uint64_t *in_b, uint32_t have, uint64_t *out, int fshift,
+__device__ __forceinline__ void msd_finish_body(const MsdArgs &a, uint32_t sb, uint64_t *buf, uint32_t *cnt, uint32_t *loff, uint32_t *wsum,
+                                                const uint64_t *in_a, uint32_t n_a, const uint64_t *in_b, uint32_t have, int fshift,
                                                 uint32_t fmask, int lowbits, uint32_t *sub, uint16_t *biglist, uint32_t *nbig_lds)
 {
     constexpr int ITEMS = CAP / THREADS;
@@ -363,6 +378,23 @@
         w[r] = j < have ? (j < n_a ? in_a[j] : in_b[j - n_a]) : ~0ull;
     }
     msd_finish_sort<CAP, THREADS>(buf, cnt, loff, wsum, w, have, fshift, fmask, lowbits, sub, biglist, nbig_lds);
+    const uint64_t o = a.off[sb];
+    uint64_t *const out = a.out + o;
+    if (a.xb) {
+        const int rest = a.kb - 2 * MSD_DIG, pb = a.pb;
+        const uint64_t top = (uint64_t)sb << (pb + rest), rmask = (1ull << rest) - 1, pmask = (1ull << pb) - 1;
+        uint8_t *const ext = a.ext + o;
+#pragma unroll
+        for (int r = 0; r < ITEMS; r++) {
+            const uint32_t j = threadIdx.x + r * THREADS;
+            if (j < have) {
+                const uint64_t y = buf[j];
+                out[j] = top | (((y >> (pb + MSD_XBITS)) & rmask) << pb) | (y & pmask);
+                ext[j] = (uint8_t)(y >> pb);
+            }
+        }
+        return;
+    }
 #pragma unroll
     for (int r = 0; r < ITEMS; r++) {
         const uint32_t j = threadIdx.x + r * THREADS;
@@ -381,8 +413,8 @@
     const uint32_t have = a.count2[blockIdx.x];
     if (have == 0 || have > MSD_FN_CAP) return;
     const uint64_t *in = a.buf2 + (uint64_t)blockIdx.x * MSD_FN_CAP;
-    msd_finish_body<MSD_FN_CAP, MSD_FN_THREADS>(buf, cnt, loff, wsum, in, have, in, have, a.out + a.off[blockIdx.x], fshift, fmask,
-                                                fshift - a.pb, sub, biglist, &nbig_lds);
+    msd_finish_body<MSD_FN_CAP, MSD_FN_THREADS>(a, blockIdx.x, buf, cnt, loff, wsum, in, have, in, have, fshift, fmask,
+                                                fshift - a.pb - a.xb, sub, biglist, &nbig_lds);
 }
 
 __global__ __launch_bounds__(MSD_BIG_THREADS) void k_msd_finish_big(MsdArgs a, const uint32_t *__restrict__ sb_sorted,
@@ -401,8 +433,8 @@
     if (e > 0 && sb_sorted[e - 1] == sb) return;
     const uint32_t have = a.count2[sb];
     if (have > MSD_BIG_CAP || have <= MSD_FN_CAP) { if (threadIdx.x == 0) atomicOr(a.flag, 16ull); return; }
-    msd_finish_body<MSD_BIG_CAP, MSD_BIG_THREADS>(buf, cnt, loff, wsum, a.buf2 + (uint64_t)sb * MSD_FN_CAP, MSD_FN_CAP, w_sorted + e, have,
-                                                  a.out + a.off[sb], fshift, fmask, fshift - a.pb, sub, biglist, &nbig_lds);
+    msd_finish_body<MSD_BIG_CAP, MSD_BIG_THREADS>(a, sb, buf, cnt, loff, wsum, a.buf2 + (uint64_t)sb * MSD_FN_CAP, MSD_FN_CAP, w_sorted + e,
+                                                  have, fshift, fmask, fshift - a.pb - a.xb, sub, biglist, &nbig_lds);
 }
 
 struct MsdPlan {
@@ -440,9 +472,12 @@
     FBG_TRY(fbg_reserve(ctx, ctx->dp_c, (nsub + 1) * 8));
     FBG_TRY(fbg_reserve(ctx, ctx->dp_d, (size_t)MSD_ARENA * 4 * 2));
     FBG_TRY(fbg_reserve(ctx, ctx->dp_e, (size_t)MSD_ARENA * 8 * 2));
+    const bool ext = ctx->opt.msd_ext != 0 && g.b == 2 && g.key_bits + MSD_XBITS + MSD_TILE_BITS <= 64 && g.K + MSD_XSYM + MSD_ITEMS - 1 <= 64;
+    if (ext) FBG_TRY(fbg_reserve(ctx, ctx->msd_ext, (size_t)N));
     unsigned long long *flag = ctx->scalars.as<unsigned long long>() + 100;
     MsdArgs &a = p->a;
     a.T = ctx->text.as<uint8_t>(); a.N = N; a.code = g.d_code; a.b = g.b; a.K = g.K; a.pb = g.pb; a.kb = g.key_bits;
+    a.xb = ext ? MSD_XBITS : 0; a.ext = ext ? ctx->msd_ext.as<uint8_t>() : nullptr;
     a.buf1 = ctx->keysA.as<uint64_t>(); a.cap1 = cap1; a.xs = xs; a.segcap = cap1 / xs;
     a.tile0 = 0; a.tiles2 = 0; a.tiles2_x = 0;
     a.count1 = ctx->dp_a.as<unsigned long long>();
@@ -490,7 +525,7 @@
     const uint64_t upto = avail >= N ? (N + MSD_TILE - 1) / MSD_TILE : (avail >= 64 ? (avail - 64) / MSD_TILE : 0);
     if (upto <= ctx->pre_tiles) return FBG_OK;
     plan.a.tile0 = ctx->pre_tiles;
-    hipLaunchKernelGGL(k_msd_pack_split, dim3((unsigned)(upto - ctx->pre_tiles)), dim3(MSD_THREADS), 0, ctx->stream, plan.a);
+    msd_launch_pass1(plan.a, (unsigned)(upto - ctx->pre_tiles), ctx->stream);
     ctx->pre_tiles = upto;
     return FBG_OK;
 }
@@ -508,6 +543,7 @@
 {
     *ok = 0;
     ctx->msd_decline = 1;
+    ctx->msd_ext_valid = false;
     const uint64_t N = ctx->N;
     hipStream_t st = ctx->stream;
     MsdPlan plan;
@@ -528,7 +564,7 @@
     unsigned long long *off = plan.off, *flag = plan.flag;
     if (!ahead) {
         FBG_TRY(fbg_stage_begin(ctx, FBG_STAGE_SORT_PASS1));
-        hipLaunchKernelGGL(k_msd_pack_split, dim3(fbg_blocks(N, MSD_TILE)), dim3(MSD_THREADS), 0, st, a);
+        msd_launch_pass1(a, fbg_blocks(N, MSD_TILE), st);
         FBG_TRY(fbg_stage_end(ctx, FBG_STAGE_SORT_PASS1, 1));
     }
     hipLaunchKernelGGL(k_msd_tiles, dim3(1), dim3(1024), 0, st, a.count1, a.segcap, nseg, tile_start, flag);
@@ -557,7 +593,7 @@
         e = rocprim::exclusive_scan(ctx->tmp.p, have, wide, off, 0ull, (size_t)nsub, rocprim::plus<unsigned long long>(), st);
         if (e != hipSuccess) return fbg_fail(ctx, FBG_ERR_HIP, "rocprim exclusive_scan: %s", hipGetErrorString(e));
     }
-    const int fshift = g.pb + rest - fbits;
+    const int fshift = g.pb + a.xb + rest - fbits;
     const uint32_t fmask = (uint32_t)((1u << fbits) - 1);
     FBG_TRY(fbg_stage_begin(ctx, FBG_STAGE_SORT_PASS3));
     hipLaunchKernelGGL(k_msd_finish, dim3((unsigned)nsub), dim3(MSD_FN_THREADS), 0, st, a, fshift, fmask);
@@ -588,6 +624,7 @@
     }
     FBG_HIP_TRY(ctx, hipGetLastError());
     *sorted = ctx->keysA.as<uint64_t>();
+    ctx->msd_ext_valid = a.xb != 0;
     *ok = 1;
     return FBG_OK;
 }
diff --git a/founderblockgraphs_amd/csrc/rank_common.h b/founderblockgraphs_amd/csrc/rank_common.h
--- a/founderblockgraphs_amd/csrc/rank_common.h
+++ b/founderblockgraphs_amd/csrc/rank_common.h
@@ -37,6 +37,8 @@
     uint32_t *tie_count;
     uint32_t tie_region;
     uint2 *pairs;
+    int pair_codes;
+    unsigned long long *pair_stats;
     uint32_t *pair_count;
     uint32_t *pm;
     uint32_t *big;
@@ -245,7 +247,8 @@
     a.b = b; a.key_bits = key_bits; a.K = K; a.reversed = ctx->reversed;
     a.gmax = ctx->gmax.as<uint32_t>();
     a.cand = nullptr; a.pm = nullptr; a.blk_count = nullptr; a.region = 0;
-    a.ties = nullptr; a.tie_count = nullptr; a.tie_region = 0; a.pairs = nullptr; a.pair_count = nullptr;
+    a.ties = nullptr; a.tie_count = nullptr; a.tie_region = 0; a.pairs = nullptr; a.pair_count = nullptr; a.pair_codes = 0;
+    a.pair_stats = nullptr;
     a.big = ctx->big_groups.as<uint32_t>();
     a.counters = ctx->scalars.as<unsigned long long>() + 32;
     a.g_min = 0;
diff --git a/founderblockgraphs_amd/csrc/rank_scan.hip b/founderblockgraphs_amd/csrc/rank_scan.hip
--- a/founderblockgraphs_amd/csrc/rank_scan.hip
+++ b/founderblockgraphs_amd/csrc/rank_scan.hip
@@ -207,6 +207,7 @@
 
 struct LeanArgs {
     const uint64_t *keys;
+    const uint8_t *ext;
     uint64_t own_lo, own_hi;
     uint32_t per_wave, pmask;
     int pb;
@@ -271,14 +272,18 @@
     const unsigned long long EVM = ((1ull << (RL_EV_HI + 1)) - 1) & ~((1ull << RL_EV_LO) - 1);
     const unsigned long long RNG = ~(1ull << 63);
     const uint64_t *__restrict__ keys = f.keys;
-    auto load_row = [&](uint32_t k0) -> uint64_t {
-        const uint32_t k = min(max(k0 - RL_EV_LO + (uint32_t)lane, own_lo), own_hi - 1);
-        return keys[k];
-    };
-    uint64_t xnext = wlo < whi ? load_row(wlo) : 0ull;
+    const uint8_t *__restrict__ ext = f.ext;
+    auto row_slot = [&](uint32_t k0) -> uint32_t { return min(max(k0 - RL_EV_LO + (uint32_t)lane, own_lo), own_hi - 1); };
+    uint64_t xnext = wlo < whi ? keys[row_slot(wlo)] : 0ull;
+    uint32_t enext = ext && wlo < whi ? ext[row_slot(wlo)] : 0u;
     for (uint32_t k0 = wlo; k0 < whi; k0 += RL_EV) {
         const uint64_t x = xnext;
-        if (k0 + RL_EV < whi) xnext = load_row(k0 + RL_EV);
+        const uint32_t ex = enext;
+        if (k0 + RL_EV < whi) {
+            const uint32_t kn = row_slot(k0 + RL_EV);
+            xnext = keys[kn];
+            if (ext) enext = ext[kn];
+        }
         const uint32_t slot = k0 - RL_EV_LO + (uint32_t)lane;
         if (k0 < own_lo + 2 * RS_HALO || k0 + RL_EV + 2 * RS_HALO > own_hi || k0 + RL_EV > whi) {
             const unsigned long long Q = EVM & __ballot(slot < whi);
@@ -311,7 +316,13 @@
                 Q = QP | (QP << 1) | (EVM & (LONG | ADJL | (~TIE & (RUN | NE))));
             }
             if (SS) {
-                if ((SS >> lane) & 1ull) my_note[nn + rl_lanes_below(SS)] = make_uint2(lo & f.pmask, lo_n & f.pmask);
+                uint32_t cx = 0, cy = 0;
+                if (ext) {
+                    const uint32_t d = (ex ^ rl_from_next(ex)) & 255u;
+                    const uint32_t c = d ? (uint32_t)(__builtin_clz(d) - 24) >> 1 : 4u;
+                    cx = c << 30; cy = (c >> 2) << 30;
+                }
+                if ((SS >> lane) & 1ull) my_note[nn + rl_lanes_below(SS)] = make_uint2((lo & f.pmask) | cx, (lo_n & f.pmask) | cy);
                 nn += (uint32_t)__popcll(SS);
             }
             if (Q) {
@@ -332,7 +343,7 @@
 {
     const uint64_t own = a.own_hi - a.own_lo, waves = (uint64_t)blocks * RL_WAVES;
     f->per_wave = (uint32_t)(((own + waves - 1) / waves + RL_EV - 1) / RL_EV * RL_EV);
-    f->keys = a.keys; f->own_lo = a.own_lo; f->own_hi = a.own_hi; f->pmask = (uint32_t)a.pmask; f->pb = pb;
+    f->keys = a.keys; f->ext = nullptr; f->own_lo = a.own_lo; f->own_hi = a.own_hi; f->pmask = (uint32_t)a.pmask; f->pb = pb;
     const double L = (double)a.row_len;
     const double delta = (ldexp(1.0, pb - 25) + ldexp(1.0, pb - 22) + 2.0) / L + 1e-6;
     f->inv_row_len = (float)(1.0 / L);
@@ -383,15 +394,35 @@
 
 __global__ __launch_bounds__(256) void k_tie_pairs(RankArgs a)
 {
+    __shared__ uint32_t s_stats[2];
     const uint32_t have = a.pair_count[blockIdx.x];
     if (have > a.tie_region) { if (threadIdx.x == 0) a.counters[1] = 1; return; }
+    if (threadIdx.x < 2) s_stats[threadIdx.x] = 0;
+    __syncthreads();
+    uint32_t n_code = 0, n_text = 0;
     for (uint32_t e = threadIdx.x; e < have; e += blockDim.x) {
-        const uint2 p = a.pairs[(size_t)blockIdx.x * a.tie_region + e];
-        const uint64_t x = fbg_load8(a.T, (uint64_t)p.x + a.K) ^ fbg_load8(a.T, (uint64_t)p.y + a.K);
-        const uint32_t h = x != 0 ? (uint32_t)(__ffsll((unsigned long long)x) - 1) / 8 : fbg_extend_match(a.T, (uint64_t)p.x + a.K, (uint64_t)p.y + a.K, 8);
+        uint2 p = a.pairs[(size_t)blockIdx.x * a.tie_region + e];
+        uint32_t h, from = (uint32_t)a.K;
+        const uint32_t c = a.pair_codes ? (p.x >> 30) | (((p.y >> 30) & 1u) << 2) : 4u;
+        if (a.pair_codes) { p.x &= 0x3fffffffu; p.y &= 0x3fffffffu; from += 4; }
+        if (c < 4) {
+            h = c;
+            n_code++;
+        } else {
+            const uint64_t x = fbg_load8(a.T, (uint64_t)p.x + from) ^ fbg_load8(a.T, (uint64_t)p.y + from);
+            h = (from - (uint32_t)a.K) +
+                (x != 0 ? (uint32_t)(__ffsll((unsigned long long)x) - 1) / 8 : fbg_extend_match(a.T, (uint64_t)p.x + from, (uint64_t)p.y + from, 8));
+            n_text++;
+        }
         const uint32_t g = fbg_clamp_lcp(h + (uint32_t)a.K) + 1;
         rs_update(a, rs_col_of_rem(a, rs_rem<FBG_SLOTS_PACKED>(a, p.x)), g);
         rs_update(a, rs_col_of_rem(a, rs_rem<FBG_SLOTS_PACKED>(a, p.y)), g);
+    }
+    if (a.pair_stats) {
+        if (n_code) atomicAdd(&s_stats[0], n_code);
+        if (n_text) atomicAdd(&s_stats[1], n_text);
+        __syncthreads();
+        if (threadIdx.x < 2 && s_stats[threadIdx.x]) atomicAdd(&a.pair_stats[threadIdx.x], (unsigned long long)s_stats[threadIdx.x]);
     }
 }
 
@@ -734,6 +765,12 @@
                       rs_lean_setup(a, a.pb, rs_blocks, &lf);
     if (lean)
     {
+        if (ctx->msd_ext_valid && a.keys == ctx->keysA.as<uint64_t>() && a.b == 2 && a.pb <= 30 && a.own_lo == 0 && a.own_hi == ctx->N) {
+            lf.ext = ctx->msd_ext.as<uint8_t>();
+            a.pair_codes = 1;
+        }
+        a.pair_stats = ctx->scalars.as<unsigned long long>() + 112;
+        FBG_HIP_TRY(ctx, hipMemsetAsync(a.pair_stats, 0, 2 * sizeof(unsigned long long), st));
         FBG_TRY(fbg_reserve(ctx, ctx->ps_g, (size_t)rs_blocks * tie_region * 8));
         FBG_TRY(fbg_reserve(ctx, ctx->ps_h, (size_t)rs_blocks * 4));
         a.pairs = ctx->ps_g.as<uint2>(); a.pair_count = ctx->ps_h.as<uint32_t>();
@@ -816,6 +853,7 @@
     *done = 0;
     ctx->ranked = false;
     ctx->part_active = false;
+    ctx->ext_pairs = ctx->text_pairs = -1;
     const uint64_t N = ctx->N, n = ctx->n;
     const int layout = rs_layout(geom);
     hipStream_t st = ctx->stream;
@@ -838,11 +876,14 @@
         launches++;
     }
     FBG_TRY(rs_join(ctx));
-    unsigned long long h[5];
+    unsigned long long h[5], ps[2] = {0, 0};
     if (a.g_min > 1)
         hipLaunchKernelGGL(k_count_unfilled, dim3(fbg_blocks(n, 256)), dim3(256), 0, st, a.gmax, n, a.g_min, a.reversed, cnt);
     FBG_HIP_TRY(ctx, hipMemcpyAsync(h, cnt, sizeof(h), hipMemcpyDeviceToHost, st));
+    if (a.pair_stats) FBG_HIP_TRY(ctx, hipMemcpyAsync(ps, a.pair_stats, sizeof(ps), hipMemcpyDeviceToHost, st));
     FBG_HIP_TRY(ctx, hipStreamSynchronize(st));
+    ctx->ext_pairs = (int64_t)ps[0];
+    ctx->text_pairs = (int64_t)ps[1];
     launches++;
     if (h[1] != 0) return fbg_stage_end(ctx, FBG_STAGE_RANKSCAN, launches);
     if (a.g_min > 1 && h[4] != 0) {
diff --git a/founderblockgraphs_amd/csrc/suffix_sort.hip b/founderblockgraphs_amd/csrc/suffix_sort.hip
--- a/founderblockgraphs_amd/csrc/suffix_sort.hip
+++ b/founderblockgraphs_amd/csrc/suffix_sort.hip
@@ -741,6 +741,7 @@
     ctx->granked = false;
     ctx->grs_ebits = nullptr;
     ctx->grs_flagged = false;
+    ctx->msd_ext_valid = false;
     KeyGeom g;
 
     if (ctx->gapfree && !ctx->have_ignore && !ctx->opt.no_ranked) {
```
